# facebookresearch/goliath

Measured on AMD Instinct MI355X. Metric: relit views/sec (fwd+bwd) at 2048x1334, 250k Gaussians, higher is better.
Workload: dtype f32; 1 GPU; rgca_config2_envrelight; gaussians=250000, views_per_gpu=8, micro_batches=2, world_size=1, dist_backend=none, rccl_world_size=0, parallelism=view-parallel x1, launch=hip_graph_replay

## Files before the change

goliath_amd/csrc/gol_raster.h:

```cpp
#pragma once
#include <type_traits>

#include "gol_common.h"

namespace {

constexpr int kBatch = 256;
constexpr float kUnA = GOL_UN_A, kUnB = GOL_UN_B;
__device__ __forceinline__ float3 true_conic(float a, float b, float c) { return make_float3(a * kUnA, b * kUnB, c * kUnA); }
#ifdef GOL_EXACT_MATH
__device__ __forceinline__ float exact_sigma(float a, float b, float c, float dx, float dy) {
#pragma clang fp contract(off)
  const float t1 = (a * dx) * dx, t2 = (c * dy) * dy, t3 = (b * dx) * dy;
  const float h = 0.5f * (t1 + t2);
  return h + t3;
}
__device__ __forceinline__ float exact_exp_neg(float s) { return (float)exp(-(double)s); }
__device__ __forceinline__ float exact_next_T(float T, float alpha) {
#pragma clang fp contract(off)
  const float om = 1.f - alpha;
  return T * om;
}
#endif

struct TileCoord { int tile, tx, ty; bool ok; };

__device__ __forceinline__ TileCoord tile_of_block(int bid, int T, int tiles_x) {
  const int tiles_y = T / tiles_x;
  const int xcd = bid & 7, j = bid >> 3;
  TileCoord tc;
  const int row_local = j / tiles_x;
  tc.tx = j - row_local * tiles_x;
  tc.ty = row_local * 8 + xcd;
  tc.ok = tc.ty < tiles_y;
  tc.tile = tc.ty * tiles_x + tc.tx;
  return tc;
}

typedef float f1 __attribute__((ext_vector_type(1)));
typedef float f2 __attribute__((ext_vector_type(2)));
typedef int i1 __attribute__((ext_vector_type(1)));
typedef int i2 __attribute__((ext_vector_type(2)));

template <int PPL> struct Pix;
template <> struct Pix<2> { typedef f2 fv; typedef i2 iv; static constexpr int kWaves = 2; };
template <> struct Pix<1> { typedef f1 fv; typedef i1 iv; static constexpr int kWaves = 4; };

template <int PPL>
__device__ __forceinline__ void wave_rect(int wave, float tile_x0, float tile_y0, float& x0, float& x1, float& y0, float& y1) {
  if (PPL == 2) {
    x0 = tile_x0 + 0.5f; x1 = x0 + 15.f; y0 = tile_y0 + (float)(wave * 8) + 0.5f; y1 = y0 + 7.f;
  } else {
    x0 = tile_x0 + (float)((wave & 1) * 8) + 0.5f; x1 = x0 + 7.f; y0 = tile_y0 + (float)((wave >> 1) * 8) + 0.5f; y1 = y0 + 7.f;
  }
}

template <int PPL>
__device__ __forceinline__ int wave_mask(float gx, float gy, float ca, float cb, float cc, float tau, float ia, float ic,
                                         float exact, float tile_x0, float tile_y0) {
  constexpr int NW = Pix<PPL>::kWaves;
  if (!(tau >= 0.f)) return 0;
  if (exact == 0.f) return (1 << NW) - 1;
  int m = 0;
#pragma unroll
  for (int q = 0; q < NW; ++q) {
    float x0, x1, y0, y1;
    wave_rect<PPL>(q, tile_x0, tile_y0, x0, x1, y0, y1);
    const float ms = gol_min_sigma_rect(gx, gy, ca, cb, cc, ia, ic, x0, x1, y0, y1);
    m |= (ms <= tau) ? (1 << q) : 0;
  }
  return m;
}

template <int PPL>
__device__ __forceinline__ void lane_pixel(int tx, int ty, int wave, int lane, int& j, int& i0) {
  if (PPL == 2) { j = tx * 16 + (lane & 15); i0 = ty * 16 + wave * 8 + (lane >> 4) * 2; }
  else { j = tx * 16 + (wave & 1) * 8 + (lane & 7); i0 = ty * 16 + (wave >> 1) * 8 + (lane >> 3); }
}

struct __attribute__((aligned(16))) StagedRow { float4 a, b; float2 c; float2 pad; };

struct Staged { float4 a, b; float2 c; int mask; };
template <int PPL>
__device__ __forceinline__ Staged stage_entry(const float* __restrict__ records, size_t g, float tile_x0, float tile_y0) {
  const float4* R = reinterpret_cast<const float4*>(records + g * GOL_SPLAT_RECORD);
  const float4 q0 = R[0], q1 = R[1], q2 = R[2], q3 = R[3];
  Staged s;
  s.a = q0;
  s.b = q1;
  s.c = make_float2(q2.x, q2.y);
  const float3 cn = true_conic(q0.z, q0.w, q1.x);
  s.mask = wave_mask<PPL>(q0.x, q0.y, cn.x, cn.y, cn.z, q2.z, q2.w, q3.x, q3.y, tile_x0, tile_y0);
  return s;
}

template <typename V, int P>
__device__ __forceinline__ bool any_live(const V& live) {
  unsigned u = 0u;
#pragma unroll
  for (int q = 0; q < P; ++q) u |= __float_as_uint(live[q]);
  return u != 0u;
}

template <int PPL> using fvec = typename Pix<PPL>::fv;
template <int PPL> using ivec = typename Pix<PPL>::iv;

template <int PPL>
__device__ __forceinline__ void visit_falloff(float ca, float cb, float cc, float dx, const fvec<PPL>& dy, fvec<PPL>& sigma,
                                              fvec<PPL>& e) {
#ifndef GOL_EXACT_MATH
  sigma = (ca * dx * dx + cc * dy * dy) + (cb * dx) * dy;
#pragma unroll
  for (int q = 0; q < PPL; ++q) e[q] = __builtin_amdgcn_exp2f(-sigma[q]);
#else
#pragma unroll
  for (int q = 0; q < PPL; ++q) { sigma[q] = exact_sigma(ca, cb, cc, dx, dy[q]); e[q] = exact_exp_neg(sigma[q]); }
#endif
}

template <int PPL>
__device__ __forceinline__ unsigned long long fwd_step(const fvec<PPL>& sigma, fvec<PPL> alpha, const fvec<PPL>& live,
                                                       const fvec<PPL>& T_cur, fvec<PPL>& vis, fvec<PPL>& next_T,
                                                       bool (&take)[PPL], unsigned long long (&stop)[PPL]) {
  alpha *= live;
  vis = alpha * T_cur;
#ifndef GOL_EXACT_MATH
  next_T = T_cur - vis;
#else
#pragma unroll
  for (int q = 0; q < PPL; ++q) next_T[q] = exact_next_T(T_cur[q], alpha[q]);
#endif
  unsigned long long any_stop = 0ull;
#pragma unroll
  for (int q = 0; q < PPL; ++q) {
    const unsigned long long mc = gol_ballot(!(sigma[q] < 0.f)) & gol_ballot(!(alpha[q] < GOL_ALPHA_FLOOR));
    const unsigned long long ms = gol_ballot(next_T[q] <= GOL_T_STOP);
    take[q] = __builtin_amdgcn_inverse_ballot_w64(mc & ~ms);
    stop[q] = mc & ms;
    any_stop |= stop[q];
  }
  return any_stop;
}

template <int PPL>
__device__ __forceinline__ void fwd_take(const bool (&take)[PPL], const fvec<PPL>& next_T, fvec<PPL>& vis, fvec<PPL>& T_cur) {
#pragma unroll
  for (int q = 0; q < PPL; ++q) vis[q] = take[q] ? vis[q] : 0.f;
#ifndef GOL_EXACT_MATH
  T_cur -= vis;
#else
#pragma unroll
  for (int q = 0; q < PPL; ++q) T_cur[q] = take[q] ? next_T[q] : T_cur[q];
#endif
}

template <int PPL>
__device__ __forceinline__ unsigned long long bwd_taken(float opacity, const fvec<PPL>& e, const fvec<PPL>& sigma, int li,
                                                        const ivec<PPL>& bin_final, fvec<PPL>& alpha,
                                                        unsigned long long (&mv)[PPL]) {
  alpha = opacity * e;
  unsigned long long many = 0ull;
#pragma unroll
  for (int q = 0; q < PPL; ++q) {
    alpha[q] = fminf(GOL_ALPHA_CAP_BWD, alpha[q]);
    mv[q] = gol_ballot(li <= bin_final[q]) & gol_ballot(!(sigma[q] < 0.f)) & gol_ballot(!(alpha[q] < GOL_ALPHA_FLOOR));
    many |= mv[q];
  }
  return many;
}

template <int PPL>
__device__ __forceinline__ void bwd_recur(const unsigned long long (&mv)[PPL], fvec<PPL>& alpha, fvec<PPL>& T_cur,
                                          bool (&v)[PPL], fvec<PPL>& ra, fvec<PPL>& fac) {
#pragma unroll
  for (int q = 0; q < PPL; ++q) {
    v[q] = __builtin_amdgcn_inverse_ballot_w64(mv[q]);
    alpha[q] = v[q] ? alpha[q] : 0.f;
  }
  const fvec<PPL> one_m = 1.f - alpha;
#pragma unroll
  for (int q = 0; q < PPL; ++q) ra[q] = __builtin_amdgcn_rcpf(one_m[q]);
  const fvec<PPL> T_new = T_cur * ra;
  fac = alpha * T_new;
  T_cur = T_new;
}

template <int PPL>
__device__ __forceinline__ void bwd_moments(const fvec<PPL>& e, const fvec<PPL>& w, const fvec<PPL>& T_cur,
                                            const fvec<PPL>& ra, const fvec<PPL>& fac, const fvec<PPL>& tail,
                                            const bool (&v)[PPL], const fvec<PPL>& dy, fvec<PPL>& qsum, fvec<PPL>& gop,
                                            fvec<PPL>& gy, fvec<PPL>& gyy) {
  const fvec<PPL> v_alpha = T_cur * w + ra * (tail - qsum);
  qsum += fac * w;
  gop = e * v_alpha;
#pragma unroll
  for (int q = 0; q < PPL; ++q) gop[q] = v[q] ? gop[q] : 0.f;
  gy = gop * dy;
  gyy = gy * dy;
}
template <int PPL>
__device__ __forceinline__ float lane_sum(const fvec<PPL>& x) {
  float s = x[0];
#pragma unroll
  for (int q = 1; q < PPL; ++q) s += x[q];
  return s;
}

template <int PPL>
__device__ __forceinline__ int wave_last_entry(const ivec<PPL>& bin_final) {
  int wmax = bin_final[0];
#pragma unroll
  for (int q = 1; q < PPL; ++q) wmax = max(wmax, bin_final[q]);
#pragma unroll
  for (int off = 32; off > 0; off >>= 1) wmax = max(wmax, __shfl_xor(wmax, off, 64));
  return __builtin_amdgcn_readfirstlane(wmax);
}

inline int64_t raster_grid(int B, int img_h, int img_w) {
  return (int64_t)B * 8 * (((img_h + 15) / 16 + 7) / 8) * ((img_w + 15) / 16);
}

#define GOL_RASTER_CHECK_DIMS(bytes_per_pixel, too_large_msg)                                                           \
  do {                                                                                                                  \
    GOL_REQUIRE(B >= 0 && N >= 0, "negative size");                                                                     \
    GOL_REQUIRE(block == 16, "only block_width == 16 is implemented (the reference's value, render_gsplat.py:28)");     \
    GOL_REQUIRE(img_h > 0 && img_w > 0, "empty image");                                                                 \
    GOL_REQUIRE(raster_grid(B, img_h, img_w) < (1ll << 31), "too many tiles");                                          \
    GOL_REQUIRE((uint64_t)img_h * (uint64_t)img_w * (uint64_t)(bytes_per_pixel) < (1ull << 32), too_large_msg);         \
  } while (0)

template <typename F>
inline void with_ppl(int ppl, F&& fn) {
  if (ppl == 2) fn(std::integral_constant<int, 2>());
  else fn(std::integral_constant<int, 1>());
}
constexpr std::true_type kYes{}; constexpr std::false_type kNo{};

}
```

goliath_amd/csrc/raster.hip:

```cpp
#include <cstdlib>

#include "gol_raster.h"

namespace {

template <bool EXTRA, bool LAZY, int PPL>
__global__ __launch_bounds__(64 * Pix<PPL>::kWaves) void raster_fwd_kernel(
    int N, int img_h, int img_w, int planar, int tiles_x, int tiles_y, const int2* __restrict__ tile_bins,
    const int32_t* __restrict__ sorted_ids, int64_t capacity, const float* __restrict__ records,
    const float* __restrict__ background, float* __restrict__ out_img,
    float* __restrict__ out_extra, float* __restrict__ final_Ts, int32_t* __restrict__ final_idx,
    float* __restrict__ out_alpha, float* __restrict__ out_extra_norm, float norm_lo,
    const float* __restrict__ l1_target, const float* __restrict__ l1_mask, int l1_mask_c,
    uint8_t* __restrict__ l1_sign, float* __restrict__ l1_partial, int n_views) {
  typedef typename Pix<PPL>::fv fv;
  typedef typename Pix<PPL>::iv iv;
  constexpr int NW = Pix<PPL>::kWaves, NT = 64 * NW;
  __shared__ float s_l1[NW];
  __shared__ float4 s_a[kBatch];
  __shared__ float4 s_b[kBatch];
  __shared__ float2 s_c[kBatch];
  __shared__ int32_t s_mask[kBatch];
  const int T = tiles_x * tiles_y;
  const int view = blockIdx.x % n_views, slot = blockIdx.x / n_views;
  const TileCoord tc = tile_of_block(slot, T, tiles_x);
  if (!tc.ok) return;
  const int tid = threadIdx.x, lane = tid & 63, wave = tid >> 6;
  int j, i0;
  lane_pixel<PPL>(tc.tx, tc.ty, wave, lane, j, i0);
  bool in[PPL];
  fv py, live;
#pragma unroll
  for (int q = 0; q < PPL; ++q) {
    in[q] = (i0 + q < img_h) && (j < img_w);
    py[q] = (float)(i0 + q) + 0.5f;
    live[q] = in[q] ? 1.f : 0.f;
  }
  const float px = (float)j + 0.5f;

  const int2 range = tile_bins[(size_t)view * T + tc.tile];
  const int32_t* ids = sorted_ids + (size_t)view * capacity;
  const size_t goff = (size_t)view * N;

  fv T_cur = 1.f;
  iv cur_idx = 0;
  fv acc0 = 0.f, acc1 = 0.f, acc2 = 0.f, acc3 = 0.f;

  const int n_batches = (range.y - range.x + kBatch - 1) / kBatch;
  for (int bb = 0; bb < n_batches; ++bb) {
    if (__syncthreads_and(!any_live<fv, PPL>(live))) break;
    const int batch_start = range.x + bb * kBatch;
    for (int k = tid; k < kBatch; k += NT) {
      const int idx = batch_start + k;
      if (idx < range.y) {
        const Staged st = stage_entry<PPL>(records, goff + (size_t)ids[idx], (float)(tc.tx * 16), (float)(tc.ty * 16));
        s_a[k] = st.a; s_b[k] = st.b; s_c[k] = st.c; s_mask[k] = st.mask;
      } else {
        s_mask[k] = 0;
      }
    }
    __syncthreads();
    const int batch_size = min(kBatch, range.y - batch_start);
    for (int chunk = 0; chunk < batch_size; chunk += 64) {
      unsigned long long bits = gol_ballot((s_mask[chunk + lane] >> wave) & 1);
      if (LAZY && gol_ballot(any_live<fv, PPL>(live)) == 0ull) break;
      while (bits) {
        if (!LAZY && gol_ballot(any_live<fv, PPL>(live)) == 0ull) { chunk = batch_size; break; }
        const int t = chunk + __builtin_ctzll(bits);
        bits &= bits - 1;
        const float4 a4 = s_a[t];
        const float4 b4 = s_b[t];
        const float2 c2 = s_c[t];
        const float dx = a4.x - px;
        const fv dy = a4.y - py;
        fv sigma, e, alpha, vis, next_T;
        visit_falloff<PPL>(a4.z, a4.w, b4.x, dx, dy, sigma, e);
#pragma unroll
        for (int q = 0; q < PPL; ++q) alpha[q] = fminf(GOL_ALPHA_CAP_FWD, b4.y * e[q]);
        bool take[PPL];
        unsigned long long stop_m[PPL];
        const unsigned long long any_stop = fwd_step<PPL>(sigma, alpha, live, T_cur, vis, next_T, take, stop_m);
        bool half_done = false;
        if (!LAZY || any_stop != 0ull) {
#pragma unroll
          for (int q = 0; q < PPL; ++q) {
            const bool stop = __builtin_amdgcn_inverse_ballot_w64(stop_m[q]);
            live[q] = stop ? 0.f : live[q];
            if (LAZY) cur_idx[q] = stop ? (batch_start + t - 1) : cur_idx[q];
          }
          if (LAZY) half_done = gol_ballot(any_live<fv, PPL>(live)) == 0ull;
        }
        fwd_take<PPL>(take, next_T, vis, T_cur);
        acc0 += b4.z * vis; acc1 += b4.w * vis; acc2 += c2.x * vis;
        if (EXTRA) acc3 += c2.y * vis;
        if (!LAZY) {
#pragma unroll
          for (int q = 0; q < PPL; ++q) cur_idx[q] = take[q] ? (batch_start + t) : cur_idx[q];
        }
        if (LAZY && half_done) { chunk = batch_size; break; }
      }
    }
  }
  if (LAZY) {
#pragma unroll
    for (int q = 0; q < PPL; ++q) cur_idx[q] = live[q] != 0.f ? range.y - 1 : cur_idx[q];
  }

  const unsigned hw = (unsigned)img_h * (unsigned)img_w;
  const size_t vplane = (size_t)view * hw;
  float* __restrict__ o_T = final_Ts + vplane;
  int32_t* __restrict__ o_idx = final_idx + vplane;
  float* __restrict__ o_img = out_img + 3 * vplane;
  float* __restrict__ o_ex = (EXTRA && out_extra) ? out_extra + vplane : nullptr;
  float* __restrict__ o_alpha = out_alpha ? out_alpha + vplane : nullptr;
  float* __restrict__ o_norm = (EXTRA && out_extra_norm) ? out_extra_norm + vplane : nullptr;
  const float* __restrict__ i_tgt = l1_target ? l1_target + 3 * vplane : nullptr;
  const float* __restrict__ i_mask = l1_mask ? l1_mask + (size_t)l1_mask_c * vplane : nullptr;
  uint8_t* __restrict__ o_sign = l1_target ? l1_sign + vplane : nullptr;
  const float bg0 = background[0], bg1 = background[1], bg2 = background[2];
  float* __restrict__ o_img1 = o_img + (planar ? hw : 1u);
  float* __restrict__ o_img2 = o_img + (planar ? 2u * hw : 2u);
  const bool bwd_state = range.y > range.x;
  float l1_acc = 0.f;
#pragma unroll
  for (int q = 0; q < PPL; ++q) {
    if (!in[q]) continue;
    const unsigned pix = (unsigned)(i0 + q) * (unsigned)img_w + (unsigned)j;
    const unsigned b4 = pix * 4u;
    const unsigned bimg = planar ? b4 : 3u * b4;
    const float Tq = T_cur[q];
    const float c0 = acc0[q] + Tq * bg0, c1 = acc1[q] + Tq * bg1, c2 = acc2[q] + Tq * bg2, ex = acc3[q];
    *gol_at(o_T, b4) = Tq;
    if (bwd_state || !LAZY) *gol_at(o_idx, b4) = cur_idx[q];
    *gol_at(o_img, bimg) = c0; *gol_at(o_img1, bimg) = c1; *gol_at(o_img2, bimg) = c2;
    if (o_ex) *gol_at(o_ex, b4) = ex;
    if (o_alpha) *gol_at(o_alpha, b4) = 1.f - Tq;
    if (o_norm) *gol_at(o_norm, b4) = ex / fminf(fmaxf(1.f - Tq, norm_lo), 1.f);
    if (i_tgt) {
      const float m0 = i_mask ? *gol_at(i_mask, b4) : 1.f;
      const float cs[3] = {c0, c1, c2};
      unsigned code = 0u;
#pragma unroll
      for (int c = 0; c < 3; ++c) {
        const float m = (i_mask && l1_mask_c == 3) ? *gol_at(i_mask + (size_t)c * hw, b4) : m0;
        const float d = (cs[c] - *gol_at(i_tgt + (size_t)c * hw, b4)) * m;
        l1_acc += fabsf(d);
        code |= (d > 0.f ? 2u : (d < 0.f ? 0u : 1u)) << (2 * c);
      }
      if (bwd_state) *gol_at(o_sign, pix) = (uint8_t)code;
    }
  }
  if (l1_target) {
    const float ws = gol_wave_sum_to_lane63(l1_acc);
    if (lane == 63) s_l1[wave] = ws;
    __syncthreads();
    if (tid == 0) {
      float tot = 0.f;
#pragma unroll
      for (int w = 0; w < NW; ++w) tot += s_l1[w];
      l1_partial[(size_t)view * T + tc.tile] = tot;
    }
  }
}

__global__ __launch_bounds__(1024) void l1_sum_kernel(int n, const float* __restrict__ l1_partial, float scale,
                                                      float* __restrict__ l1_out) {
  __shared__ float s_w[16];
  float a0 = 0.f, a1 = 0.f, a2 = 0.f, a3 = 0.f;
  const int n4 = n >> 2;
  const float4* p4 = reinterpret_cast<const float4*>(l1_partial);
  int i = threadIdx.x;
  for (; i + 3 * 1024 < n4; i += 4 * 1024) {
    const float4 v0 = p4[i], v1 = p4[i + 1024], v2 = p4[i + 2048], v3 = p4[i + 3072];
    a0 += (v0.x + v0.y) + (v0.z + v0.w); a1 += (v1.x + v1.y) + (v1.z + v1.w);
    a2 += (v2.x + v2.y) + (v2.z + v2.w); a3 += (v3.x + v3.y) + (v3.z + v3.w);
  }
  for (; i < n4; i += 1024) { const float4 v = p4[i]; a0 += (v.x + v.y) + (v.z + v.w); }
  if ((int)threadIdx.x < (n & 3)) a1 += l1_partial[4 * n4 + threadIdx.x];
  const float ws = gol_wave_sum_to_lane63((a0 + a1) + (a2 + a3));
  if ((threadIdx.x & 63) == 63) s_w[threadIdx.x >> 6] = ws;
  __syncthreads();
  if (threadIdx.x == 0) {
    float tot = 0.f;
#pragma unroll
    for (int w = 0; w < 16; ++w) tot += s_w[w];
    l1_out[0] = tot * scale;
  }
}

constexpr int kBatchB = 64;
constexpr int kAcc = 12;

static_assert(kBatchB == 64, "raster_bwd_kernel ballots one 64-entry chunk per batch");

template <bool EXTRA, bool PACKED, int PPL>
__global__ __launch_bounds__(64 * Pix<PPL>::kWaves) void raster_bwd_kernel(
    int N, int img_h, int img_w, int planar, int tiles_x, int tiles_y, const int2* __restrict__ tile_bins,
    const int32_t* __restrict__ sorted_ids, int64_t capacity, const float* __restrict__ records,
    const float* __restrict__ background,
    const float* __restrict__ final_Ts, const int32_t* __restrict__ final_idx,
    const float* __restrict__ v_out_img, const float* __restrict__ v_out_extra,
    const float* __restrict__ v_out_alpha, float* __restrict__ v_xy, float* __restrict__ v_conic,
    float* __restrict__ v_colors, float* __restrict__ v_extra, float* __restrict__ v_opacity,
    const uint8_t* __restrict__ v_sign, const float* __restrict__ v_sign_mask, int v_sign_mask_c,
    const float* __restrict__ v_img_scale, float v_img_scale_mul, int n_views) {
  typedef typename Pix<PPL>::fv fv;
  typedef typename Pix<PPL>::iv iv;
  constexpr int NW = Pix<PPL>::kWaves, NT = 64 * NW;
  __shared__ StagedRow s_e[kBatchB];
  __shared__ int32_t s_mask[kBatchB];
  __shared__ int32_t s_id[kBatchB];
  __shared__ __attribute__((aligned(16))) float s_acc[NW][kBatchB][kAcc];
  __shared__ int32_t s_touched[NW][kBatchB];
  __shared__ int32_t s_wmax[NW];
  const int T = tiles_x * tiles_y;
  const int view = blockIdx.x % n_views, slot = blockIdx.x / n_views;
  const TileCoord tc = tile_of_block(slot, T, tiles_x);
  if (!tc.ok) return;
  const int2 range = tile_bins[(size_t)view * T + tc.tile];
  if (range.y <= range.x) return;
  const int tid = threadIdx.x, lane = tid & 63, wave = tid >> 6;
  int j, i0;
  lane_pixel<PPL>(tc.tx, tc.ty, wave, lane, j, i0);
  const float px = (float)j + 0.5f;
  const size_t hw = (size_t)img_h * img_w;
  const int32_t* ids = sorted_ids + (size_t)view * capacity;
  const size_t goff = (size_t)view * N;
  bool in[PPL];
  size_t pp[PPL];
  fv py, T_final;
  iv bin_final;
#pragma unroll
  for (int q = 0; q < PPL; ++q) {
    in[q] = (i0 + q < img_h) && (j < img_w);
    py[q] = (float)(i0 + q) + 0.5f;
    pp[q] = in[q] ? ((size_t)view * img_h + i0 + q) * img_w + j : 0;
    T_final[q] = in[q] ? final_Ts[pp[q]] : 1.f;
    bin_final[q] = in[q] ? final_idx[pp[q]] : (range.x - 1);
  }
  fv T_cur = T_final;
  fv vo0 = 0.f, vo1 = 0.f, vo2 = 0.f, vo3 = 0.f, voa = 0.f;
  {
    const float vsc = (v_img_scale ? v_img_scale[0] : 1.f) * v_img_scale_mul;
    const size_t os = planar ? hw : 1;
#pragma unroll
    for (int q = 0; q < PPL; ++q) {
      if (!in[q]) continue;
      const size_t p = pp[q];
      const int i = i0 + q;
      const size_t o = planar ? (size_t)view * 3 * hw + (size_t)i * img_w + j : 3 * p;
      float g0 = 0.f, g1 = 0.f, g2 = 0.f;
      if (v_out_img) { g0 = v_out_img[o]; g1 = v_out_img[o + os]; g2 = v_out_img[o + 2 * os]; }
      if (v_sign) {
        const unsigned code = v_sign[p];
        float m0 = vsc, m1 = vsc, m2 = vsc;
        if (v_sign_mask) {
          const float* mk = v_sign_mask + (size_t)view * v_sign_mask_c * hw + (size_t)i * img_w + j;
          m0 *= mk[0]; m1 *= (v_sign_mask_c == 3) ? mk[hw] : mk[0]; m2 *= (v_sign_mask_c == 3) ? mk[2 * hw] : mk[0];
        }
        g0 += (float)((int)(code & 3u) - 1) * m0;
        g1 += (float)((int)((code >> 2) & 3u) - 1) * m1;
        g2 += (float)((int)((code >> 4) & 3u) - 1) * m2;
      }
      vo0[q] = g0; vo1[q] = g1; vo2[q] = g2;
      if (EXTRA && v_out_extra) vo3[q] = v_out_extra[p];
      if (v_out_alpha) voa[q] = v_out_alpha[p];
    }
  }
  const fv tail = T_final * (voa - (background[0] * vo0 + background[1] * vo1 + background[2] * vo2));
  fv qsum = 0.f;

  const int wmax = wave_last_entry<PPL>(bin_final);
  if (lane == 0) s_wmax[wave] = wmax;
  __syncthreads();
  int bmax = s_wmax[0];
#pragma unroll
  for (int w = 1; w < NW; ++w) bmax = max(bmax, s_wmax[w]);
  bmax = min(bmax, range.y - 1);
  if (bmax < range.x) return;

  float* acc_lane = &s_acc[wave][0][lane >> 4];
  const int n_batches = (bmax - range.x + kBatchB) / kBatchB;
  auto entry_id = [&](int bb2) {
    const int e = bmax - bb2 * kBatchB - tid;
    return (tid < kBatchB && e >= range.x) ? ids[e] : 0;
  };
  int gid_next = entry_id(0);
  for (int bb = 0; bb < n_batches; ++bb) {
    __syncthreads();
    const int batch_end = bmax - bb * kBatchB;
    const int batch_size = min(kBatchB, batch_end + 1 - range.x);
    const int gid = gid_next;
    if (tid < kBatchB) {
      if (tid < batch_size) {
        const Staged st = stage_entry<PPL>(records, goff + (size_t)gid, (float)(tc.tx * 16), (float)(tc.ty * 16));
        s_e[tid].a = st.a; s_e[tid].b = st.b; s_e[tid].c = st.c; s_mask[tid] = st.mask;
        s_id[tid] = gid;
      } else {
        s_mask[tid] = 0;
      }
    }
    if (bb + 1 < n_batches) gid_next = entry_id(bb + 1);
    (&s_touched[0][0])[tid] = 0;
    __syncthreads();

    const int t0 = max(0, batch_end - wmax);
    unsigned long long bits = gol_ballot((s_mask[lane] >> wave) & 1);
    if (t0 > 0) bits &= ~0ull << t0;
    while (bits) {
      const int t = __builtin_ctzll(bits);
      bits &= bits - 1;
      const float4 a4 = s_e[t].a;
      const float4 b4 = s_e[t].b;
      const float2 c2 = s_e[t].c;
      const int li = batch_end - t;
      const float dx = a4.x - px;
      const fv dy = a4.y - py;
      fv sigma, vis, alpha, ra, fac;
      visit_falloff<PPL>(a4.z, a4.w, b4.x, dx, dy, sigma, vis);
      unsigned long long mv[PPL];
      if (bwd_taken<PPL>(b4.y, vis, sigma, li, bin_final, alpha, mv) == 0ull) continue;
      bool v[PPL];
      bwd_recur<PPL>(mv, alpha, T_cur, v, ra, fac);
      fv w = b4.z * vo0 + b4.w * vo1 + c2.x * vo2;
      if (EXTRA) w += c2.y * vo3;
      fv gop, gy, gyy;
      bwd_moments<PPL>(vis, w, T_cur, ra, fac, tail, v, dy, qsum, gop, gy, gyy);
      float g0s, g1s, g2s, g3 = 0.f;
      if (PPL == 2) {
        g0s = __builtin_fmaf(fac[0], vo0[0], fac[PPL - 1] * vo0[PPL - 1]);
        g1s = __builtin_fmaf(fac[0], vo1[0], fac[PPL - 1] * vo1[PPL - 1]);
        g2s = __builtin_fmaf(fac[0], vo2[0], fac[PPL - 1] * vo2[PPL - 1]);
        if (EXTRA) g3 = __builtin_fmaf(fac[0], vo3[0], fac[PPL - 1] * vo3[PPL - 1]);
      } else {
        g0s = fac[0] * vo0[0]; g1s = fac[0] * vo1[0]; g2s = fac[0] * vo2[0];
        if (EXTRA) g3 = fac[0] * vo3[0];
      }
      const float m0 = lane_sum<PPL>(gop), my = lane_sum<PPL>(gy), myy = lane_sum<PPL>(gyy);
      const float mx = m0 * dx, mxx = mx * dx, mxy = my * dx;
      const float r0 = gol_wave_sum4(g0s, g1s, g2s, m0);
      const float r1 = gol_wave_sum4(mx, my, mxx, mxy);
      const float r2 = gol_wave_sum_to_lane63(myy);
      const float r3 = EXTRA ? gol_wave_sum_to_lane63(g3) : 0.f;
      if ((lane & 15) == 15) {
        float* a = gol_at(acc_lane, (unsigned)t * (unsigned)(kAcc * sizeof(float)));
        a[0] = r0; a[4] = r1;
        if (lane == 63) { a[8 - 3] = r2; a[9 - 3] = r3; }
        s_touched[wave][t] = 1;
      }
    }
    __syncthreads();
    if (PACKED) {
      float* rec = v_colors;
      for (int idx = tid; idx < batch_size * 16; idx += NT) {
        const int t = idx >> 4, c = idx & 15;
        bool any = false;
#pragma unroll
        for (int w = 0; w < NW; ++w) any = any || (s_touched[w][t] != 0);
        if (!any || c > (EXTRA ? 9 : 8)) continue;
        const float4 a4 = s_e[t].a;
        const float4 b4 = s_e[t].b;
        const float nop = -b4.y, cc = b4.x;
        const int k1 = (c == 5) ? 4 : c, k2 = 5;
        const float w1 = (c == 4) ? nop * a4.z * kUnA : (c == 5) ? nop * a4.w * kUnB : (c == 6 || c == 8) ? 0.5f * nop
                       : (c == 7) ? nop : 1.f;
        const float w2 = (c == 4) ? nop * a4.w * kUnB : (c == 5) ? nop * cc * kUnA : 0.f;
        float s1 = 0.f, s2 = 0.f;
#pragma unroll
        for (int w = 0; w < NW; ++w) {
          const bool tw = s_touched[w][t] != 0;
          s1 += tw ? s_acc[w][t][k1] : 0.f;
          s2 += tw ? s_acc[w][t][k2] : 0.f;
        }
        atomicAdd(rec + (goff + (size_t)s_id[t]) * 16 + c, w1 * s1 + w2 * s2);
      }
    } else if (tid < batch_size) {
      float a[kAcc];
#pragma unroll
      for (int k = 0; k < kAcc; ++k) a[k] = 0.f;
      bool any = false;
#pragma unroll
      for (int w = 0; w < NW; ++w) {
        if (s_touched[w][tid]) {
          any = true;
          const float4* q = reinterpret_cast<const float4*>(&s_acc[w][tid][0]);
          const float4 q0 = q[0], q1 = q[1], q2 = q[2];
          a[0] += q0.x; a[1] += q0.y; a[2] += q0.z; a[3] += q0.w;
          a[4] += q1.x; a[5] += q1.y; a[6] += q1.z; a[7] += q1.w;
          a[8] += q2.x; a[9] += q2.y;
        }
      }
      if (any) {
        const size_t g = goff + (size_t)s_id[tid];
        const float4 a4 = s_e[tid].a;
        const float4 b4 = s_e[tid].b;
        const float nop = -b4.y;
        const float3 cn = true_conic(a4.z, a4.w, b4.x);
        atomicAdd(v_colors + 3 * g, a[0]); atomicAdd(v_colors + 3 * g + 1, a[1]); atomicAdd(v_colors + 3 * g + 2, a[2]);
        atomicAdd(v_opacity + g, a[3]);
        atomicAdd(v_xy + 2 * g, nop * (cn.x * a[4] + cn.y * a[5]));
        atomicAdd(v_xy + 2 * g + 1, nop * (cn.y * a[4] + cn.z * a[5]));
        atomicAdd(v_conic + 3 * g, 0.5f * nop * a[6]); atomicAdd(v_conic + 3 * g + 1, nop * a[7]);
        atomicAdd(v_conic + 3 * g + 2, 0.5f * nop * a[8]);
        if (EXTRA && v_extra) atomicAdd(v_extra + g, a[9]);
      }
    }
  }
}

__global__ __launch_bounds__(256) void raster_count_pairs_kernel(int N, int img_h, int img_w, int tiles_x, int tiles_y,
                                                                 const int2* __restrict__ tile_bins,
                                                                 const int32_t* __restrict__ sorted_ids, int64_t capacity,
                                                                 const float* __restrict__ records,
                                                                 const int32_t* __restrict__ final_idx,
                                                                 unsigned long long* __restrict__ counts) {
  __shared__ unsigned long long s_cnt[2];
  const int view = blockIdx.y, tile = blockIdx.x, T = tiles_x * tiles_y;
  const int ty = tile / tiles_x, tx = tile - ty * tiles_x;
  const int j = tx * 16 + (threadIdx.x & 15), i = ty * 16 + (threadIdx.x >> 4);
  if (threadIdx.x < 2) s_cnt[threadIdx.x] = 0ull;
  __syncthreads();
  const int2 range = tile_bins[(size_t)view * T + tile];
  unsigned long long tested = 0, taken = 0;
  if (i < img_h && j < img_w && range.y > range.x) {
    const int last = min(range.y - 1, final_idx[((size_t)view * img_h + i) * img_w + j]);
    const float px = (float)j + 0.5f, py = (float)i + 0.5f;
    for (int li = range.x; li <= last; ++li) {
      const float4* R = reinterpret_cast<const float4*>(records + ((size_t)view * N + sorted_ids[(size_t)view * capacity + li]) * GOL_SPLAT_RECORD);
      const float4 q0 = R[0], q1 = R[1];
      const float dx = q0.x - px, dy = q0.y - py;
      f1 sg, e;
      visit_falloff<1>(q0.z, q0.w, q1.x, dx, f1(dy), sg, e);
      const float alpha = fminf(GOL_ALPHA_CAP_FWD, q1.y * e[0]);
      ++tested;
      taken += (!(sg[0] < 0.f) && !(alpha < GOL_ALPHA_FLOOR)) ? 1 : 0;
    }
  }
  atomicAdd(&s_cnt[0], tested);
  atomicAdd(&s_cnt[1], taken);
  __syncthreads();
  if (threadIdx.x < 2 && s_cnt[threadIdx.x]) atomicAdd(counts + 2 * view + threadIdx.x, s_cnt[threadIdx.x]);
}

__global__ __launch_bounds__(256) void splat_pack_kernel(size_t n, const float* __restrict__ xys,
                                                         const float* __restrict__ conics,
                                                         const float* __restrict__ colors,
                                                         const float* __restrict__ extra,
                                                         const float* __restrict__ opacities,
                                                         float* __restrict__ records) {
  const size_t e = (size_t)blockIdx.x * 256 + threadIdx.x;
  if (e >= n) return;
  gol_record_write(records + e * GOL_SPLAT_RECORD, xys[2 * e], xys[2 * e + 1], conics[3 * e], conics[3 * e + 1],
                   conics[3 * e + 2], opacities[e], colors ? colors[3 * e] : 0.f, colors ? colors[3 * e + 1] : 0.f,
                   colors ? colors[3 * e + 2] : 0.f, extra ? extra[e] : 0.f);
}

}

extern "C" int gol_raster_plan(int B, int* fwd_pixels_per_lane) {
  static const int forced = getenv("GOL_RASTER_PPL") ? atoi(getenv("GOL_RASTER_PPL")) : 0;
  if (fwd_pixels_per_lane) *fwd_pixels_per_lane = (forced == 1 || forced == 2) ? forced : (B <= 2 ? 1 : 2);
  return GOL_OK;
}

extern "C" int gol_raster_count_pairs(int B, int N, int img_h, int img_w, const int32_t* tile_bins, const int32_t* sorted_ids,
                                      int64_t capacity, const float* records, const int32_t* final_idx, uint64_t* counts,
                                      void* stream) {
  GOL_REQUIRE(B >= 0 && N >= 0 && img_h > 0 && img_w > 0, "bad size");
  if (B == 0) return GOL_OK;
  GOL_REQUIRE(tile_bins && final_idx && counts && (capacity == 0 || sorted_ids) && (N == 0 || records), "null pointer");
  hipStream_t s = (hipStream_t)stream;
  if (hipMemsetAsync(counts, 0, sizeof(uint64_t) * 2 * (size_t)B, s) != hipSuccess) {
    gol_set_error("gol_raster_count_pairs: hipMemsetAsync failed");
    return GOL_ERR_LAUNCH;
  }
  const int tiles_x = (img_w + 15) / 16, tiles_y = (img_h + 15) / 16;
  raster_count_pairs_kernel<<<dim3(tiles_x * tiles_y, B), 256, 0, s>>>(
      N, img_h, img_w, tiles_x, tiles_y, reinterpret_cast<const int2*>(tile_bins), sorted_ids, capacity, records, final_idx,
      reinterpret_cast<unsigned long long*>(counts));
  GOL_CHECK_LAUNCH();
  return GOL_OK;
}

extern "C" int gol_splat_pack(int B, int N, const float* xys, const float* conics, const float* colors,
                              const float* extra, const float* opacities, float* records, void* stream) {
  GOL_REQUIRE(B >= 0 && N >= 0, "negative size");
  if (B == 0 || N == 0) return GOL_OK;
  GOL_REQUIRE(xys && conics && opacities && records, "null pointer");
  const size_t n = (size_t)B * N;
  splat_pack_kernel<<<gol_cdiv((long long)n, 256), 256, 0, (hipStream_t)stream>>>(n, xys, conics, colors, extra, opacities,
                                                                                 records);
  GOL_CHECK_LAUNCH();
  return GOL_OK;
}

extern "C" int gol_rasterize_fwd(int B, int N, int img_h, int img_w, int block, int planar, const int32_t* tile_bins,
                                 const int32_t* sorted_ids, int64_t capacity, const float* records, int with_extra,
                                 const float* background, float* out_img,
                                 float* out_extra, float* final_Ts, int32_t* final_idx, float* out_alpha,
                                 float* out_extra_norm, float norm_lo, const float* l1_target, const float* l1_mask,
                                 int l1_mask_c, uint8_t* l1_sign, float* l1_partial, float* l1_out, float l1_scale,
                                 int pixels_per_lane, void* stream) {
  GOL_RASTER_CHECK_DIMS(12, "image too large (32-bit byte offsets inside a view)");
  if (B == 0) return GOL_OK;
  GOL_REQUIRE(tile_bins && background && out_img && final_Ts && final_idx, "null pointer");
  GOL_REQUIRE(capacity == 0 || sorted_ids, "null sorted_ids");
  GOL_REQUIRE(N == 0 || records, "null Gaussian records");
  GOL_REQUIRE((!out_extra && !out_extra_norm) || with_extra || N == 0, "out_extra / out_extra_norm need the extra channel");
  GOL_REQUIRE(!with_extra || out_extra || out_extra_norm, "extra without an output for it");
  GOL_REQUIRE(!l1_target || (planar && l1_sign && l1_partial), "the fused L1 needs planar images, l1_sign and l1_partial");
  GOL_REQUIRE(!l1_mask || (l1_target && (l1_mask_c == 1 || l1_mask_c == 3)), "l1_mask: 1 or 3 channels, with l1_target");
  GOL_REQUIRE(!l1_out || l1_target, "l1_out needs l1_target");
  const int tiles_x = (img_w + 15) / 16, tiles_y = (img_h + 15) / 16;
  const dim3 grid((unsigned)raster_grid(B, img_h, img_w));
  const int2* bins = reinterpret_cast<const int2*>(tile_bins);
  hipStream_t s = (hipStream_t)stream;
  GOL_REQUIRE(pixels_per_lane >= 0 && pixels_per_lane <= 2, "pixels_per_lane: 0 (choose by B), 1 or 2");
  int ppl = pixels_per_lane;
  if (ppl == 0) gol_raster_plan(B, &ppl);
  auto launch = [&](auto ex_c, auto lazy_c) {
    with_ppl(ppl, [&](auto ppl_c) {
      constexpr bool EX = decltype(ex_c)::value, LZ = decltype(lazy_c)::value;
      constexpr int PPL = decltype(ppl_c)::value;
      raster_fwd_kernel<EX, LZ, PPL><<<grid, 64 * Pix<PPL>::kWaves, 0, s>>>(
          N, img_h, img_w, planar, tiles_x, tiles_y, bins, sorted_ids, capacity, records, background, out_img, out_extra,
          final_Ts, final_idx, out_alpha, EX ? out_extra_norm : nullptr, norm_lo, l1_target, l1_mask, l1_mask_c, l1_sign,
          l1_partial, B);
    });
  };
  const bool ex = out_extra || out_extra_norm;
  if (ex && planar) launch(kYes, kYes);
  else if (ex) launch(kYes, kNo);
  else if (planar) launch(kNo, kYes);
  else launch(kNo, kNo);
  if (l1_out) l1_sum_kernel<<<1, 1024, 0, s>>>(B * tiles_x * tiles_y, l1_partial, l1_scale, l1_out);
  GOL_CHECK_LAUNCH();
  return GOL_OK;
}

extern "C" int gol_rasterize_bwd(int B, int N, int img_h, int img_w, int block, int planar, const int32_t* tile_bins,
                                 const int32_t* sorted_ids, int64_t capacity, const float* records, int with_extra,
                                 const float* background, const float* final_Ts,
                                 const int32_t* final_idx, const float* v_out_img, const float* v_out_extra,
                                 const float* v_out_alpha, float* v_xy, float* v_conic, float* v_colors,
                                 float* v_extra, float* v_opacity, int grad_stride, const uint8_t* v_sign,
                                 const float* v_sign_mask, int v_sign_mask_c, const float* v_img_scale,
                                 float v_img_scale_mul, int pixels_per_lane, void* stream) {
  GOL_RASTER_CHECK_DIMS(0, "");
  if (B == 0 || N == 0 || capacity == 0) return GOL_OK;
  GOL_REQUIRE(tile_bins && sorted_ids && background && final_Ts && final_idx, "null pointer");
  GOL_REQUIRE(v_out_img || v_sign, "no upstream image gradient (v_out_img or v_sign)");
  GOL_REQUIRE(!v_sign || planar, "the sign image of the fused L1 goes with planar images");
  GOL_REQUIRE(!v_sign_mask || (v_sign && (v_sign_mask_c == 1 || v_sign_mask_c == 3)), "v_sign_mask: 1 or 3 channels, with v_sign");
  GOL_REQUIRE(records, "null Gaussian records");
  GOL_REQUIRE(v_xy && v_conic && v_colors && v_opacity, "null gradient output");
  GOL_REQUIRE(!(v_out_extra || v_extra) || with_extra, "extra-channel gradients need the extra channel");
  GOL_REQUIRE(grad_stride == 0 || grad_stride == GOL_GRAD_RECORD, "grad_stride must be 0 (dense arrays) or 16 (records)");
  const bool packed = grad_stride == GOL_GRAD_RECORD;
  if (packed)
    GOL_REQUIRE(v_opacity == v_colors + 3 && v_xy == v_colors + 4 && v_conic == v_colors + 6 &&
                    (!v_extra || v_extra == v_colors + 9),
                "record layout is [rgb | opacity | xy | conic | extra | pad] (GOL_GRAD_RECORD floats)");
  const int tiles_x = (img_w + 15) / 16, tiles_y = (img_h + 15) / 16;
  const dim3 grid((unsigned)raster_grid(B, img_h, img_w));
  const int2* bins = reinterpret_cast<const int2*>(tile_bins);
  hipStream_t s = (hipStream_t)stream;
  GOL_REQUIRE(pixels_per_lane >= 0 && pixels_per_lane <= 2, "pixels_per_lane: 0 (2), 1 or 2");
  const int ppl = pixels_per_lane ? pixels_per_lane : 2;
  const bool ex = with_extra && (v_out_extra || v_extra);
  auto launch = [&](auto ex_c, auto packed_c) {
    with_ppl(ppl, [&](auto ppl_c) {
      constexpr bool EX = decltype(ex_c)::value, PK = decltype(packed_c)::value;
      constexpr int PPL = decltype(ppl_c)::value;
      raster_bwd_kernel<EX, PK, PPL><<<grid, 64 * Pix<PPL>::kWaves, 0, s>>>(
          N, img_h, img_w, planar, tiles_x, tiles_y, bins, sorted_ids, capacity, records, background, final_Ts, final_idx,
          v_out_img, EX ? v_out_extra : nullptr, v_out_alpha, v_xy, v_conic, v_colors, EX ? v_extra : nullptr, v_opacity,
          v_sign, v_sign_mask, v_sign_mask_c, v_img_scale, v_img_scale_mul, B);
    });
  };
  if (ex && packed) launch(kYes, kYes);
  else if (ex) launch(kYes, kNo);
  else if (packed) launch(kNo, kYes);
  else launch(kNo, kNo);
  GOL_CHECK_LAUNCH();
  return GOL_OK;
}
```

goliath_amd/csrc/raster_nd.hip:

```cpp
#include "gol_raster.h"

namespace {

constexpr int kChunkMax = 16;
constexpr int kBatchNdB = 64;

template <int CK>
__device__ __forceinline__ void stage_colors(float* __restrict__ row, const float* __restrict__ colors, size_t g, int C,
                                             int c0, int nc) {
  const float* col = colors + g * (size_t)C + c0;
#pragma unroll
  for (int c = 0; c < CK; ++c) row[c] = (c < nc) ? col[c] : 0.f;
}

template <int CK, int PPL>
__global__ __launch_bounds__(64 * Pix<PPL>::kWaves) void raster_nd_fwd_kernel(
    int N, int C, int c_first, int img_h, int img_w, int tiles_x, int tiles_y, const int2* __restrict__ tile_bins,
    const int32_t* __restrict__ sorted_ids, int64_t capacity, const float* __restrict__ records,
    const float* __restrict__ colors, const float* __restrict__ background, float* __restrict__ out_img,
    float* __restrict__ final_Ts, int32_t* __restrict__ final_idx, int n_views) {
  typedef typename Pix<PPL>::fv fv;
  typedef typename Pix<PPL>::iv iv;
  constexpr int NW = Pix<PPL>::kWaves, NT = 64 * NW;
  __shared__ float4 s_a[kBatch];
  __shared__ float2 s_b[kBatch];
  __shared__ int32_t s_mask[kBatch];
  __shared__ __attribute__((aligned(16))) float s_col[kBatch * CK];
  const int T = tiles_x * tiles_y;
  const int view = blockIdx.x % n_views, slot = blockIdx.x / n_views;
  const TileCoord tc = tile_of_block(slot, T, tiles_x);
  if (!tc.ok) return;
  const int c0 = c_first + (int)blockIdx.y * CK;
  const int nc = min(CK, C - c0);
  const int tid = threadIdx.x, lane = tid & 63, wave = tid >> 6;
  int j, i0;
  lane_pixel<PPL>(tc.tx, tc.ty, wave, lane, j, i0);
  bool in[PPL];
  fv py, live;
#pragma unroll
  for (int q = 0; q < PPL; ++q) {
    in[q] = (i0 + q < img_h) && (j < img_w);
    py[q] = (float)(i0 + q) + 0.5f;
    live[q] = in[q] ? 1.f : 0.f;
  }
  const float px = (float)j + 0.5f;

  const int2 range = tile_bins[(size_t)view * T + tc.tile];
  const int32_t* ids = sorted_ids + (size_t)view * capacity;
  const size_t goff = (size_t)view * N;

  fv T_cur = 1.f;
  iv cur_idx = 0;
  fv acc[CK];
#pragma unroll
  for (int c = 0; c < CK; ++c) acc[c] = 0.f;

  const int n_batches = (range.y - range.x + kBatch - 1) / kBatch;
  for (int bb = 0; bb < n_batches; ++bb) {
    if (__syncthreads_and(!any_live<fv, PPL>(live))) break;
    const int batch_start = range.x + bb * kBatch;
    for (int k = tid; k < kBatch; k += NT) {
      const int idx = batch_start + k;
      if (idx < range.y) {
        const size_t g = goff + (size_t)ids[idx];
        const Staged st = stage_entry<PPL>(records, g, (float)(tc.tx * 16), (float)(tc.ty * 16));
        s_a[k] = st.a; s_b[k] = make_float2(st.b.x, st.b.y); s_mask[k] = st.mask;
        stage_colors<CK>(s_col + k * CK, colors, g, C, c0, nc);
      } else {
        s_mask[k] = 0;
      }
    }
    __syncthreads();
    const int batch_size = min(kBatch, range.y - batch_start);
    for (int chunk = 0; chunk < batch_size; chunk += 64) {
      unsigned long long bits = gol_ballot((s_mask[chunk + lane] >> wave) & 1);
      while (bits) {
        if (gol_ballot(any_live<fv, PPL>(live)) == 0ull) { chunk = batch_size; break; }
        const int t = chunk + __builtin_ctzll(bits);
        bits &= bits - 1;
        const float4 a4 = s_a[t];
        const float2 b2 = s_b[t];
        const float dx = a4.x - px;
        const fv dy = a4.y - py;
        fv sigma, e, alpha, vis, next_T;
        visit_falloff<PPL>(a4.z, a4.w, b2.x, dx, dy, sigma, e);
#pragma unroll
        for (int q = 0; q < PPL; ++q) alpha[q] = fminf(GOL_ALPHA_CAP_FWD, b2.y * e[q]);
        bool take[PPL];
        unsigned long long stop_m[PPL];
        fwd_step<PPL>(sigma, alpha, live, T_cur, vis, next_T, take, stop_m);
#pragma unroll
        for (int q = 0; q < PPL; ++q) live[q] = __builtin_amdgcn_inverse_ballot_w64(stop_m[q]) ? 0.f : live[q];
        fwd_take<PPL>(take, next_T, vis, T_cur);
        const float* col = s_col + t * CK;
#pragma unroll
        for (int c = 0; c < CK; ++c) acc[c] += col[c] * vis;
#pragma unroll
        for (int q = 0; q < PPL; ++q) cur_idx[q] = take[q] ? (batch_start + t) : cur_idx[q];
      }
    }
  }

  const unsigned hw = (unsigned)img_h * (unsigned)img_w;
  const size_t vplane = (size_t)view * hw;
  float* __restrict__ o_img = out_img + (size_t)C * vplane + c0;
  float* __restrict__ o_T = final_Ts + vplane;
  int32_t* __restrict__ o_idx = final_idx + vplane;
  const bool first = c0 == 0;
  float bg[CK];
#pragma unroll
  for (int c = 0; c < CK; ++c) bg[c] = (c < nc) ? background[c0 + c] : 0.f;
#pragma unroll
  for (int q = 0; q < PPL; ++q) {
    if (!in[q]) continue;
    const unsigned pix = (unsigned)(i0 + q) * (unsigned)img_w + (unsigned)j;
    const float Tq = T_cur[q];
    if (first) { *gol_at(o_T, pix * 4u) = Tq; *gol_at(o_idx, pix * 4u) = cur_idx[q]; }
    const unsigned bimg = pix * (unsigned)C * 4u;
#pragma unroll
    for (int c = 0; c < CK; ++c)
      if (c < nc) *gol_at(o_img + c, bimg) = acc[c][q] + Tq * bg[c];
  }
}

template <int CK, int PPL>
__global__ __launch_bounds__(64 * Pix<PPL>::kWaves) void raster_nd_bwd_kernel(
    int N, int C, int c_first, int img_h, int img_w, int tiles_x, int tiles_y, const int2* __restrict__ tile_bins,
    const int32_t* __restrict__ sorted_ids, int64_t capacity, const float* __restrict__ records,
    const float* __restrict__ colors, const float* __restrict__ background, const float* __restrict__ final_Ts,
    const int32_t* __restrict__ final_idx, const float* __restrict__ v_out_img, const float* __restrict__ v_out_alpha,
    float* __restrict__ v_xy, float* __restrict__ v_conic, float* __restrict__ v_colors, float* __restrict__ v_opacity,
    int n_views) {
  typedef typename Pix<PPL>::fv fv;
  typedef typename Pix<PPL>::iv iv;
  constexpr int NW = Pix<PPL>::kWaves, NT = 64 * NW;
  constexpr int NS = CK + 6, NG = (NS + 3) / 4, kRow = 4 * NG;
  static_assert(NW * kBatchNdB == NT, "s_touched is cleared one element per thread");
  __shared__ float4 s_a[kBatchNdB];
  __shared__ float2 s_b[kBatchNdB];
  __shared__ int32_t s_mask[kBatchNdB];
  __shared__ int32_t s_id[kBatchNdB];
  __shared__ __attribute__((aligned(16))) float s_col[kBatchNdB * CK];
  __shared__ __attribute__((aligned(16))) float s_acc[NW][kBatchNdB][kRow];
  __shared__ int32_t s_touched[NW][kBatchNdB];
  __shared__ int32_t s_wmax[NW];
  const int T = tiles_x * tiles_y;
  const int view = blockIdx.x % n_views, slot = blockIdx.x / n_views;
  const TileCoord tc = tile_of_block(slot, T, tiles_x);
  if (!tc.ok) return;
  const int2 range = tile_bins[(size_t)view * T + tc.tile];
  if (range.y <= range.x) return;
  const int c0 = c_first + (int)blockIdx.y * CK;
  const int nc = min(CK, C - c0);
  const int tid = threadIdx.x, lane = tid & 63, wave = tid >> 6;
  int j, i0;
  lane_pixel<PPL>(tc.tx, tc.ty, wave, lane, j, i0);
  const float px = (float)j + 0.5f;
  const int32_t* ids = sorted_ids + (size_t)view * capacity;
  const size_t goff = (size_t)view * N;
  fv py, T_final, voa = 0.f;
  iv bin_final;
  fv vo[CK];
#pragma unroll
  for (int c = 0; c < CK; ++c) vo[c] = 0.f;
#pragma unroll
  for (int q = 0; q < PPL; ++q) {
    const bool in = (i0 + q < img_h) && (j < img_w);
    py[q] = (float)(i0 + q) + 0.5f;
    const size_t p = in ? ((size_t)view * img_h + i0 + q) * img_w + j : 0;
    T_final[q] = in ? final_Ts[p] : 1.f;
    bin_final[q] = in ? final_idx[p] : (range.x - 1);
    if (in) {
      const float* g = v_out_img + p * (size_t)C + c0;
#pragma unroll
      for (int c = 0; c < CK; ++c) vo[c][q] = (c < nc) ? g[c] : 0.f;
      if (v_out_alpha && c0 == 0) voa[q] = v_out_alpha[p];
    }
  }

  const int wmax = wave_last_entry<PPL>(bin_final);
  if (lane == 0) s_wmax[wave] = wmax;
  __syncthreads();
  int bmax = s_wmax[0];
#pragma unroll
  for (int w = 1; w < NW; ++w) bmax = max(bmax, s_wmax[w]);
  bmax = min(bmax, range.y - 1);
  if (bmax < range.x) return;

  fv bgdot = 0.f;
#pragma unroll
  for (int c = 0; c < CK; ++c) bgdot += ((c < nc) ? background[c0 + c] : 0.f) * vo[c];
  const fv tail = T_final * (voa - bgdot);
  fv T_cur = T_final;
  fv qsum = 0.f;

  float* acc_lane = &s_acc[wave][0][lane >> 4];
  const int n_batches = (bmax - range.x + kBatchNdB) / kBatchNdB;
  for (int bb = 0; bb < n_batches; ++bb) {
    __syncthreads();
    const int batch_end = bmax - bb * kBatchNdB;
    const int batch_size = min(kBatchNdB, batch_end + 1 - range.x);
    if (tid < kBatchNdB) {
      if (tid < batch_size) {
        const int gid = ids[batch_end - tid];
        const size_t g = goff + (size_t)gid;
        const Staged st = stage_entry<PPL>(records, g, (float)(tc.tx * 16), (float)(tc.ty * 16));
        s_a[tid] = st.a; s_b[tid] = make_float2(st.b.x, st.b.y); s_mask[tid] = st.mask;
        s_id[tid] = gid;
        stage_colors<CK>(s_col + tid * CK, colors, g, C, c0, nc);
      } else {
        s_mask[tid] = 0;
      }
    }
    (&s_touched[0][0])[tid] = 0;
    __syncthreads();

    const int t0 = max(0, batch_end - wmax);
    unsigned long long bits = gol_ballot((s_mask[lane] >> wave) & 1);
    if (t0 > 0) bits &= ~0ull << t0;
    while (bits) {
      const int t = __builtin_ctzll(bits);
      bits &= bits - 1;
      const float4 a4 = s_a[t];
      const float2 b2 = s_b[t];
      const int li = batch_end - t;
      const float dx = a4.x - px;
      const fv dy = a4.y - py;
      fv sigma, vis, alpha, ra, fac;
      visit_falloff<PPL>(a4.z, a4.w, b2.x, dx, dy, sigma, vis);
      unsigned long long mv[PPL];
      if (bwd_taken<PPL>(b2.y, vis, sigma, li, bin_final, alpha, mv) == 0ull) continue;
      bool v[PPL];
      bwd_recur<PPL>(mv, alpha, T_cur, v, ra, fac);
      const float* col = s_col + t * CK;
      fv w = 0.f;
#pragma unroll
      for (int c = 0; c < CK; ++c) w += col[c] * vo[c];
      fv gop, gy, gyy;
      bwd_moments<PPL>(vis, w, T_cur, ra, fac, tail, v, dy, qsum, gop, gy, gyy);
      float s[kRow];
#pragma unroll
      for (int c = 0; c < CK; ++c) {
        s[c] = fac[0] * vo[c][0];
#pragma unroll
        for (int q = 1; q < PPL; ++q) s[c] = __builtin_fmaf(fac[q], vo[c][q], s[c]);
      }
      const float m0 = lane_sum<PPL>(gop), my = lane_sum<PPL>(gy), myy = lane_sum<PPL>(gyy);
      const float mx = m0 * dx;
      s[CK + 0] = m0; s[CK + 1] = mx; s[CK + 2] = my; s[CK + 3] = mx * dx; s[CK + 4] = my * dx; s[CK + 5] = myy;
#pragma unroll
      for (int k = NS; k < kRow; ++k) s[k] = 0.f;
      float r[NG];
#pragma unroll
      for (int gi = 0; gi < NG; ++gi) r[gi] = gol_wave_sum4(s[4 * gi], s[4 * gi + 1], s[4 * gi + 2], s[4 * gi + 3]);
      if ((lane & 15) == 15) {
        float* a = gol_at(acc_lane, (unsigned)t * (unsigned)(kRow * sizeof(float)));
#pragma unroll
        for (int gi = 0; gi < NG; ++gi) a[4 * gi] = r[gi];
        s_touched[wave][t] = 1;
      }
    }
    __syncthreads();
    for (int idx = tid; idx < batch_size * NS; idx += NT) {
      const int t = idx / NS, k = idx - t * NS;
      if (k < CK && k >= nc) continue;
      bool any = false;
#pragma unroll
      for (int w = 0; w < NW; ++w) any = any || (s_touched[w][t] != 0);
      if (!any) continue;
      const size_t g = goff + (size_t)s_id[t];
      const float4 a4 = s_a[t];
      const float2 b2 = s_b[t];
      const float nop = -b2.y;
      const float3 cn = true_conic(a4.z, a4.w, b2.x);
      const float ca = cn.x, cb = cn.y, cc = cn.z;
      int k1 = k, k2 = k;
      float w1 = 1.f, w2 = 0.f;
      float* dst;
      if (k < CK) {
        dst = v_colors + g * (size_t)C + c0 + k;
      } else {
        const int m = k - CK;
        k1 = (m == 1 || m == 2) ? CK + 1 : k;
        k2 = CK + 2;
        w1 = (m == 0) ? 1.f : (m == 1) ? nop * ca : (m == 2) ? nop * cb : (m == 4) ? nop : 0.5f * nop;
        w2 = (m == 1) ? nop * cb : (m == 2) ? nop * cc : 0.f;
        dst = (m == 0) ? v_opacity + g : (m <= 2) ? v_xy + 2 * g + (m - 1) : v_conic + 3 * g + (m - 3);
      }
      float s1 = 0.f, s2 = 0.f;
#pragma unroll
      for (int w = 0; w < NW; ++w) {
        const bool tw = s_touched[w][t] != 0;
        s1 += tw ? s_acc[w][t][k1] : 0.f;
        s2 += tw ? s_acc[w][t][k2] : 0.f;
      }
      atomicAdd(dst, w1 * s1 + w2 * s2);
    }
  }
}

struct NdPlan { int n16, tail, tail_first; };
NdPlan nd_plan(int C) {
  const int r = C % kChunkMax;
  NdPlan p;
  p.n16 = C / kChunkMax + (r > 8 ? 1 : 0);
  p.tail = (r == 0 || r > 8) ? 0 : r <= 1 ? 1 : r <= 2 ? 2 : r <= 4 ? 4 : 8;
  p.tail_first = (C / kChunkMax) * kChunkMax;
  return p;
}

template <typename F>
bool for_nd_launches(int C, F&& fn) {
  const NdPlan pl = nd_plan(C);
  if (pl.n16 > 0) fn(std::integral_constant<int, 16>(), pl.n16, 0);
  switch (pl.tail) {
    case 0: break;
    case 1: fn(std::integral_constant<int, 1>(), 1, pl.tail_first); break;
    case 2: fn(std::integral_constant<int, 2>(), 1, pl.tail_first); break;
    case 4: fn(std::integral_constant<int, 4>(), 1, pl.tail_first); break;
    case 8: fn(std::integral_constant<int, 8>(), 1, pl.tail_first); break;
    default: return false;
  }
  return true;
}

}

extern "C" int gol_rasterize_nd_fwd(int B, int N, int C, int img_h, int img_w, int block, const int32_t* tile_bins,
                                    const int32_t* sorted_ids, int64_t capacity, const float* records, const float* colors,
                                    const float* background, float* out_img, float* final_Ts, int32_t* final_idx,
                                    int pixels_per_lane, void* stream) {
  GOL_REQUIRE(C >= 1, "C >= 1 colour channels");
  GOL_REQUIRE(C <= 16 * 65535, "too many colour channels (at most 1048560: one launch row of 16-channel chunks)");
  GOL_RASTER_CHECK_DIMS((uint64_t)C * 4ull, "image too large (32-bit byte offsets inside a view: H * W * C * 4 bytes)");
  if (B == 0) return GOL_OK;
  GOL_REQUIRE(tile_bins && background && out_img && final_Ts && final_idx, "null pointer");
  GOL_REQUIRE(capacity == 0 || sorted_ids, "null sorted_ids");
  GOL_REQUIRE(N == 0 || (records && colors), "null Gaussian records / colors");
  GOL_REQUIRE(pixels_per_lane >= 0 && pixels_per_lane <= 2, "pixels_per_lane: 0 (choose by B), 1 or 2");
  int ppl = pixels_per_lane;
  if (ppl == 0) gol_raster_plan(B, &ppl);
  const int tiles_x = (img_w + 15) / 16, tiles_y = (img_h + 15) / 16;
  const unsigned gx = (unsigned)raster_grid(B, img_h, img_w);
  const int2* bins = reinterpret_cast<const int2*>(tile_bins);
  hipStream_t s = (hipStream_t)stream;
  const bool covered = for_nd_launches(C, [&](auto ck_c, int n_chunks, int c_first) {
    with_ppl(ppl, [&](auto ppl_c) {
      constexpr int CK = decltype(ck_c)::value, PPL = decltype(ppl_c)::value;
      raster_nd_fwd_kernel<CK, PPL><<<dim3(gx, n_chunks), 64 * Pix<PPL>::kWaves, 0, s>>>(
          N, C, c_first, img_h, img_w, tiles_x, tiles_y, bins, sorted_ids, capacity, records, colors, background, out_img,
          final_Ts, final_idx, B);
    });
  });
  GOL_REQUIRE(covered, "no kernel instance for this chunk width");
  GOL_CHECK_LAUNCH();
  return GOL_OK;
}

extern "C" int gol_rasterize_nd_bwd(int B, int N, int C, int img_h, int img_w, int block, const int32_t* tile_bins,
                                    const int32_t* sorted_ids, int64_t capacity, const float* records, const float* colors,
                                    const float* background, const float* final_Ts, const int32_t* final_idx,
                                    const float* v_out_img, const float* v_out_alpha, float* v_xy, float* v_conic,
                                    float* v_colors, float* v_opacity, void* stream) {
  GOL_REQUIRE(C >= 1, "C >= 1 colour channels");
  GOL_REQUIRE(C <= 16 * 65535, "too many colour channels (at most 1048560: one launch row of 16-channel chunks)");
  GOL_RASTER_CHECK_DIMS((uint64_t)C * 4ull, "image too large (32-bit byte offsets inside a view: H * W * C * 4 bytes)");
  if (B == 0 || N == 0 || capacity == 0) return GOL_OK;
  GOL_REQUIRE(tile_bins && sorted_ids && background && final_Ts && final_idx, "null pointer");
  GOL_REQUIRE(v_out_img, "null v_out_img");
  GOL_REQUIRE(records && colors, "null Gaussian records / colors");
  GOL_REQUIRE(v_xy && v_conic && v_colors && v_opacity, "null gradient output");
  const int tiles_x = (img_w + 15) / 16, tiles_y = (img_h + 15) / 16;
  const unsigned gx = (unsigned)raster_grid(B, img_h, img_w);
  const int2* bins = reinterpret_cast<const int2*>(tile_bins);
  hipStream_t s = (hipStream_t)stream;
  const bool covered = for_nd_launches(C, [&](auto ck_c, int n_chunks, int c_first) {
    constexpr int CK = decltype(ck_c)::value;
    raster_nd_bwd_kernel<CK, 2><<<dim3(gx, n_chunks), 128, 0, s>>>(
        N, C, c_first, img_h, img_w, tiles_x, tiles_y, bins, sorted_ids, capacity, records, colors, background, final_Ts,
        final_idx, v_out_img, v_out_alpha, v_xy, v_conic, v_colors, v_opacity, B);
  });
  GOL_REQUIRE(covered, "no kernel instance for this chunk width");
  GOL_CHECK_LAUNCH();
  return GOL_OK;
}
```

goliath_amd/csrc/render.hip:

```cpp
#include <cstring>

#include "gol_common.h"

namespace {
inline int64_t align256(int64_t x) { return (x + 255) & ~(int64_t)255; }
template <typename T>
inline T* at(void* ws, int64_t off) { return reinterpret_cast<T*>(reinterpret_cast<char*>(ws) + off); }
}

static int render_layout(int B, int N, int img_h, int img_w, int64_t capacity, int with_l1, bool projected, gol_render_ws* L) {
  GOL_REQUIRE(B >= 0 && N >= 0 && img_h > 0 && img_w > 0 && capacity >= 0 && L != nullptr, "bad argument");
  const int64_t T = (int64_t)((img_w + 15) / 16) * ((img_h + 15) / 16), P = (int64_t)img_h * img_w;
  const int64_t BN = (int64_t)B * N, cap = capacity > 0 ? capacity : 1;
  int64_t o = 0;
  auto take = [&](int64_t bytes) { const int64_t at_ = o; o = align256(o + bytes); return at_; };
  L->cov3d = -1;
  L->xys = projected ? -1 : take(BN * 2 * 4);
  L->depths = projected ? -1 : take(BN * 4);
  L->radii = projected ? -1 : take(BN * 4);
  L->conics = projected ? -1 : take(BN * 3 * 4);
  L->comp = projected ? -1 : take(BN * 4);
  L->nth = -1;
  L->opac_eff = projected ? -1 : take(BN * 4);
  L->records = projected ? -1 : take(BN * GOL_SPLAT_RECORD * 4);
  L->tile_count = take((int64_t)B * T * 4);
  L->tile_bins = take((int64_t)B * T * 2 * 4);
  L->keys = take((int64_t)B * cap * 8);
  L->sorted_ids = take((int64_t)B * cap * 4);
  L->n_isect = take((int64_t)B * 4);
  L->final_T = take((int64_t)B * P * 4);
  L->final_idx = take((int64_t)B * P * 4);
  L->l1_sign = with_l1 ? take((int64_t)B * P) : -1;
  L->total = o;
  return GOL_OK;
}

extern "C" int gol_render_layout(int B, int N, int img_h, int img_w, int64_t capacity, int with_l1, gol_render_ws* L) {
  return render_layout(B, N, img_h, img_w, capacity, with_l1, false, L);
}

extern "C" int gol_render_layout_projected(int B, int N, int img_h, int img_w, int64_t capacity, int with_l1,
                                           gol_render_ws* L) {
  return render_layout(B, N, img_h, img_w, capacity, with_l1, true, L);
}

static int render_fwd_from(int B, int N, int img_h, int img_w, const float* xys, const float* depths, const int32_t* radii,
                           const float* conics, const float* opac_eff, const float* records, const float* background,
                           int with_depth, float norm_lo, int64_t capacity, void* ws, const gol_render_ws* L,
                           float* out_img, float* out_depth, float* out_alpha, float* out_depth_norm,
                           const float* l1_target, const float* l1_mask, int l1_mask_c, float* l1_partial, float* l1_out,
                           float l1_scale, void* stream) {
  int rc = gol_bin_sort(B, N, xys, depths, radii, conics, opac_eff, img_h, img_w, 16, capacity,
                        at<int32_t>(ws, L->tile_count), at<int32_t>(ws, L->tile_bins), at<uint64_t>(ws, L->keys),
                        at<int32_t>(ws, L->sorted_ids), at<int32_t>(ws, L->n_isect), nullptr, stream);
  if (rc != GOL_OK) return rc;
  return gol_rasterize_fwd(B, N, img_h, img_w, 16, 1, at<int32_t>(ws, L->tile_bins), at<int32_t>(ws, L->sorted_ids),
                           capacity, records, with_depth ? 1 : 0, background, out_img,
                           with_depth ? out_depth : nullptr, at<float>(ws, L->final_T), at<int32_t>(ws, L->final_idx),
                           out_alpha, with_depth ? out_depth_norm : nullptr, norm_lo, l1_target, l1_mask, l1_mask_c,
                           l1_target ? at<uint8_t>(ws, L->l1_sign) : nullptr, l1_partial, l1_out, l1_scale, 0,
                           stream);
}

static int render_bwd_to_records(int B, int N, int img_h, int img_w, const float* records, const float* background,
                                 int64_t capacity, void* ws, const gol_render_ws* L, const float* v_img,
                                 const float* v_depth, const float* v_alpha, int use_l1_sign, const float* l1_mask,
                                 int l1_mask_c, const float* v_img_scale, float v_img_scale_mul, float* grad_records,
                                 void* stream) {
  hipStream_t s = (hipStream_t)stream;
  if (hipMemsetAsync(grad_records, 0, sizeof(float) * (size_t)B * N * GOL_GRAD_RECORD, s) != hipSuccess) {
    gol_set_error("gol_render_bwd: hipMemsetAsync failed");
    return GOL_ERR_LAUNCH;
  }
  float* g = grad_records;
  const bool use_depth = v_depth != nullptr;
  return gol_rasterize_bwd(B, N, img_h, img_w, 16, 1, at<int32_t>(ws, L->tile_bins), at<int32_t>(ws, L->sorted_ids),
                           capacity, records, use_depth ? 1 : 0, background,
                           at<float>(ws, L->final_T), at<int32_t>(ws, L->final_idx), v_img, v_depth, v_alpha, g + 4, g + 6,
                           g, use_depth ? g + 9 : nullptr, g + 3, GOL_GRAD_RECORD,
                           use_l1_sign ? at<uint8_t>(ws, L->l1_sign) : nullptr, use_l1_sign ? l1_mask : nullptr,
                           use_l1_sign ? l1_mask_c : 0, v_img_scale, v_img_scale_mul, 0, stream);
}

extern "C" int gol_render_fwd(int B, int N, int img_h, int img_w, float glob_scale, float clip_thresh, const float* means,
                              const float* scales, const float* quats, const float* opacity, const float* colors,
                              const float* viewmats, const float* intrins, const float* background, int with_depth,
                              float norm_lo, int64_t capacity, void* workspace, const gol_render_ws* L, float* out_img,
                              float* out_depth, float* out_alpha, float* out_depth_norm, const float* l1_target,
                              const float* l1_mask, int l1_mask_c, float* l1_partial, float* l1_out, float l1_scale,
                              void* stream) {
  GOL_REQUIRE(workspace != nullptr && L != nullptr, "null workspace / layout");
  GOL_REQUIRE(!l1_target || L->l1_sign >= 0, "layout was computed without the fused L1");
  if (B == 0) return GOL_OK;
  void* ws = workspace;
  GOL_REQUIRE(!l1_out || l1_target, "l1_out needs l1_target");
  int rc = gol_project_fwd(B, N, means, scales, glob_scale, quats, viewmats, intrins, img_h, img_w, 16, clip_thresh,
                           nullptr, at<float>(ws, L->xys), at<float>(ws, L->depths),
                           at<int32_t>(ws, L->radii), at<float>(ws, L->conics), at<float>(ws, L->comp),
                           nullptr, opacity, at<float>(ws, L->opac_eff), colors,
                           at<float>(ws, L->records), stream);
  if (rc != GOL_OK) return rc;
  return render_fwd_from(B, N, img_h, img_w, at<float>(ws, L->xys), at<float>(ws, L->depths), at<int32_t>(ws, L->radii),
                         at<float>(ws, L->conics), at<float>(ws, L->opac_eff), at<float>(ws, L->records), background,
                         with_depth, norm_lo, capacity, ws, L, out_img, out_depth, out_alpha, out_depth_norm, l1_target,
                         l1_mask, l1_mask_c, l1_partial, l1_out, l1_scale, stream);
}

extern "C" int gol_render_fwd_projected(int B, int N, const gol_shade_proj* proj, const float* background, int with_depth,
                                        float norm_lo, int64_t capacity, void* workspace, const gol_render_ws* L,
                                        float* out_img, float* out_depth, float* out_alpha, float* out_depth_norm,
                                        const float* l1_target, const float* l1_mask, int l1_mask_c, float* l1_partial,
                                        float* l1_out, float l1_scale, void* stream) {
  GOL_REQUIRE(workspace != nullptr && L != nullptr && proj != nullptr, "null workspace / layout / projection");
  GOL_REQUIRE(!l1_target || L->l1_sign >= 0, "layout was computed without the fused L1");
  GOL_REQUIRE(!l1_out || l1_target, "l1_out needs l1_target");
  if (B == 0) return GOL_OK;
  return render_fwd_from(B, N, proj->img_h, proj->img_w, proj->xys, proj->depths, proj->radii, proj->conics,
                         proj->opac_eff, proj->records, background, with_depth, norm_lo, capacity, workspace, L, out_img,
                         out_depth, out_alpha, out_depth_norm, l1_target, l1_mask, l1_mask_c, l1_partial, l1_out,
                         l1_scale, stream);
}

extern "C" int gol_render_bwd(int B, int N, int img_h, int img_w, float glob_scale, const float* means,
                              const float* scales, const float* quats, const float* opacity, const float* viewmats,
                              const float* intrins, const float* background, int64_t capacity, void* workspace,
                              const gol_render_ws* L, const float* v_img, const float* v_depth, const float* v_alpha,
                              int use_l1_sign, const float* l1_mask, int l1_mask_c, const float* v_img_scale,
                              float v_img_scale_mul, float* grad_records, float* v_mean, float* v_scale, float* v_quat, float* v_opacity,
                              float* v_colors, void* stream) {
  GOL_REQUIRE(workspace != nullptr && L != nullptr && grad_records != nullptr, "null workspace / layout / gradient records");
  GOL_REQUIRE(!use_l1_sign || L->l1_sign >= 0, "layout was computed without the fused L1");
  if (B == 0 || N == 0) return GOL_OK;
  void* ws = workspace;
  const float* g = grad_records;
  const bool use_depth = v_depth != nullptr;
  int rc = render_bwd_to_records(B, N, img_h, img_w, at<float>(ws, L->records), background, capacity, ws, L, v_img, v_depth,
                                 v_alpha, use_l1_sign, l1_mask, l1_mask_c, v_img_scale, v_img_scale_mul, grad_records,
                                 stream);
  if (rc != GOL_OK) return rc;
  return gol_project_bwd_records(B, N, means, scales, glob_scale, quats, viewmats, intrins, at<int32_t>(ws, L->radii),
                                 at<float>(ws, L->conics), at<float>(ws, L->comp), opacity, g, use_depth ? 1 : 0, v_mean,
                                 v_scale, v_quat, v_opacity, v_colors, stream);
}

extern "C" int gol_render_bwd_projected(int B, int N, const gol_shade_proj* proj, const float* background, int64_t capacity,
                                        void* workspace, const gol_render_ws* L, const float* v_img, const float* v_depth,
                                        const float* v_alpha, int use_l1_sign, const float* l1_mask, int l1_mask_c,
                                        const float* v_img_scale, float v_img_scale_mul, float* grad_records,
                                        void* stream) {
  GOL_REQUIRE(workspace != nullptr && L != nullptr && proj != nullptr && grad_records != nullptr,
              "null workspace / layout / projection / gradient records");
  GOL_REQUIRE(!use_l1_sign || L->l1_sign >= 0, "layout was computed without the fused L1");
  if (B == 0 || N == 0) return GOL_OK;
  return render_bwd_to_records(B, N, proj->img_h, proj->img_w, proj->records, background, capacity, workspace, L, v_img,
                               v_depth, v_alpha, use_l1_sign, l1_mask, l1_mask_c, v_img_scale, v_img_scale_mul,
                               grad_records, stream);
}
```

goliath_amd/splat.py:

```python
import ctypes
import math
import os

import torch

from . import _lib, views as _views
from ._lib import c_float, c_i64, c_int, fptr, ptr, stream_ptr

BLOCK = 16
GRAD_RECORD = 16
SPLAT_RECORD = 16

def _tiles(img_h, img_w, block=BLOCK):
    return ((img_w + block - 1) // block) * ((img_h + block - 1) // block)


class CapacityPlanner:

    def __init__(self):
        self.capacity = {}
        self.mode = os.environ.get("GOLIATH_CAPACITY_MODE", "adaptive")
        self.pending = []
        self.frozen = False
        self.frozen_log = []
        self.reruns = 0
        self.truncated = 0
        self.last_worst = {}
        self.force_block = set()
        self._pinned = {}

    def check_frozen(self):
        for n_isect, capacity in self.frozen_log:
            worst = int(n_isect.max()) if n_isect.numel() else 0
            if worst > capacity:
                raise _lib.GoliathHipError(f"a captured render_views call overflowed its intersection capacity "
                                           f"({worst} > {capacity}): re-capture with a larger capacity")

    def must_block(self, key):
        if self.mode == "verify" or os.environ.get("GOLIATH_STRICT_CAPACITY", "0") == "1":
            return True
        if self.mode == "async":
            return False
        seen, cap = self.last_worst.get(key), self.capacity.get(key)
        return key in self.force_block or seen is None or cap is None or seen * 1.5 > cap

    def passed(self, key):
        self.force_block.discard(key)

    def get(self, key):
        return self.capacity.get(key)

    def initial(self, N, T):
        return int(min(2**31 - 1, max(1 << 16, 16 * N + T)))

    def set(self, key, counts_max):
        want = int(min(2**31 - 1, max(1 << 16, int(counts_max * 2.0) + 4096)))
        self.capacity[key] = max(self.capacity.get(key, 0), want)
        return self.capacity[key]

    def observe(self, key, worst, capacity):
        self.last_worst[key] = worst
        if key not in self.capacity or worst * 1.5 > capacity:
            self.set(key, worst)

    def _take_pinned(self, B):
        free = self._pinned.setdefault(B, [])
        return free.pop() if free else torch.empty(B, dtype=torch.int32, pin_memory=True)

    def fetch(self, n_isect):
        B = n_isect.numel()
        host = self._take_pinned(B)
        host.copy_(n_isect, non_blocking=True)
        ev = torch.cuda.Event()
        ev.record()
        return host, ev

    def finish(self, host, ev):
        ev.synchronize()
        worst = int(host.max()) if host.numel() else 0
        self._pinned[host.numel()].append(host)
        return worst

    def note(self, key, n_isect, capacity):
        host, ev = self.fetch(n_isect)
        self.pending.append((ev, host, capacity, key))

    def poll(self, block=False):
        still, overflow = [], None
        for ev, host, capacity, key in self.pending:
            if block:
                ev.synchronize()
            if ev.query():
                worst = int(host.max()) if host.numel() else 0
                self._pinned[host.numel()].append(host)
                if worst > capacity:
                    self.last_worst[key] = worst
                    self.set(key, worst)
                    self.force_block.add(key)
                    overflow = (worst, capacity, key)
                else:
                    self.observe(key, worst, capacity)
            else:
                still.append((ev, host, capacity, key))
        self.pending = still
        if overflow is not None:
            worst, capacity, key = overflow
            msg = (f"a previous render_views call overflowed its intersection capacity ({worst} > {capacity}): its tile "
                   f"lists were truncated. Capacity was raised to {self.capacity[key]}")
            if self.mode == "async":
                raise _lib.GoliathHipError(msg + " -- re-run the step (GOLIATH_CAPACITY_MODE=verify repairs inside the "
                                                 "call instead).")
            import sys
            import warnings

            self.truncated += 1
            try:
                frame = sys._getframe(2)
            except ValueError:
                frame = sys._getframe(0)
            warnings.warn_explicit(msg + "; calls of this shape check their own counts before returning until one has passed "
                                         "(GOLIATH_CAPACITY_MODE=verify checks every call).", CapacityWarning,
                                   frame.f_code.co_filename, frame.f_lineno, module=frame.f_globals.get("__name__"), registry={})


class CapacityWarning(RuntimeWarning):
    """A render_views call was found, after the fact, to have rendered with truncated tile lists (adaptive mode)."""


PLANNER = CapacityPlanner()


class _Workspace:

    def __init__(self, B, N, T, capacity, device):
        self.capacity = capacity
        self.tile_count = torch.zeros(B, T, dtype=torch.int32, device=device)
        self.tile_bins = torch.empty(B, T, 2, dtype=torch.int32, device=device)
        self.keys = torch.empty(B, max(capacity, 1), dtype=torch.int64, device=device)
        self.sorted_ids = torch.empty(B, max(capacity, 1), dtype=torch.int32, device=device)
        self.n_isect = torch.empty(B, dtype=torch.int32, device=device)
        self.reach = torch.empty(B, max(N, 1), dtype=torch.int64, device=device)


_F32, _I32, _I64, _U8 = torch.float32, torch.int32, torch.int64, torch.uint8


def _p(x, dtype=_F32, name="tensor"):
    return ctypes.c_void_p(x) if x is None or isinstance(x, int) else ptr(x, dtype, name)


def _abi_bin_sort(*, B, N, xys, depths, radii, conics=None, opacities=None, img_h, img_w, capacity, tile_count, tile_bins,
                  isect_keys, sorted_ids, n_isect, reach_scratch=None):
    _lib.call("gol_bin_sort", c_int(B), c_int(N), _p(xys), _p(depths), _p(radii, _I32), _p(conics), _p(opacities),
              c_int(img_h), c_int(img_w), c_int(BLOCK), c_i64(capacity), _p(tile_count, _I32), _p(tile_bins, _I32),
              _p(isect_keys, _I64), _p(sorted_ids, _I32), _p(n_isect, _I32), _p(reach_scratch, _I64), stream_ptr())


def _abi_project_fwd(*, B, N, means3d, scales, glob_scale, quats, viewmats, intrins, img_h, img_w, clip_thresh, cov3d=None,
                     xys, depths, radii, conics, compensation, num_tiles_hit=None, opacities=None, opac_eff=None,
                     colors=None, records=None):
    _lib.call("gol_project_fwd", c_int(B), c_int(N), _p(means3d, name="means3d"), _p(scales, name="scales"),
              c_float(glob_scale), _p(quats, name="quats"), _p(viewmats, name="viewmat"), _p(intrins, name="intrins"),
              c_int(img_h), c_int(img_w), c_int(BLOCK), c_float(clip_thresh), _p(cov3d), _p(xys), _p(depths),
              _p(radii, _I32), _p(conics), _p(compensation), _p(num_tiles_hit, _I32), _p(opacities, name="opacity"),
              _p(opac_eff), _p(colors, name="colors"), _p(records), stream_ptr())


def _abi_project_bwd(*, B, N, means3d, scales, glob_scale, quats, viewmats, intrins, cov3d=None, radii, conics, compensation,
                     v_xy=None, v_depth=None, v_conic=None, v_compensation=None, opacities=None, v_opac_eff=None,
                     grad_stride=0, v_mean3d, v_scale, v_quat, v_opacity=None):
    _lib.call("gol_project_bwd", c_int(B), c_int(N), _p(means3d), _p(scales), c_float(glob_scale), _p(quats),
              _p(viewmats), _p(intrins), _p(cov3d), _p(radii, _I32), _p(conics), _p(compensation), _p(v_xy), _p(v_depth),
              _p(v_conic), _p(v_compensation), _p(opacities), _p(v_opac_eff), c_int(grad_stride), _p(v_mean3d),
              _p(v_scale), _p(v_quat), _p(v_opacity), stream_ptr())


def _abi_rasterize_fwd(*, B, N, img_h, img_w, planar, tile_bins, sorted_ids, capacity, records, with_extra, background,
                       out_img, out_extra=None, final_Ts, final_idx, out_alpha=None, out_extra_norm=None, norm_lo=0.0,
                       l1_target=None, l1_mask=None, l1_mask_c=0, l1_sign=None, l1_partial=None, l1_out=None,
                       l1_scale=1.0, pixels_per_lane=0):
    _lib.call("gol_rasterize_fwd", c_int(B), c_int(N), c_int(img_h), c_int(img_w), c_int(BLOCK), c_int(planar),
              _p(tile_bins, _I32), _p(sorted_ids, _I32), c_i64(capacity), _p(records), c_int(with_extra),
              _p(background), _p(out_img), _p(out_extra), _p(final_Ts), _p(final_idx, _I32), _p(out_alpha),
              _p(out_extra_norm), c_float(norm_lo), _p(l1_target), _p(l1_mask), c_int(l1_mask_c), _p(l1_sign, _U8),
              _p(l1_partial), _p(l1_out), c_float(l1_scale), c_int(pixels_per_lane), stream_ptr())


def _abi_rasterize_bwd(*, B, N, img_h, img_w, planar, tile_bins, sorted_ids, capacity, records, with_extra, background,
                       final_Ts, final_idx, v_out_img=None, v_out_extra=None, v_out_alpha=None, v_xy, v_conic, v_colors,
                       v_extra=None, v_opacity, grad_stride=0, v_sign=None, v_sign_mask=None, v_sign_mask_c=0,
                       v_img_scale=None, v_img_scale_mul=1.0, pixels_per_lane=0):
    _lib.call("gol_rasterize_bwd", c_int(B), c_int(N), c_int(img_h), c_int(img_w), c_int(BLOCK), c_int(planar),
              _p(tile_bins, _I32), _p(sorted_ids, _I32), c_i64(capacity), _p(records), c_int(with_extra), _p(background),
              _p(final_Ts), _p(final_idx, _I32), _p(v_out_img), _p(v_out_extra), _p(v_out_alpha), _p(v_xy), _p(v_conic),
              _p(v_colors), _p(v_extra), _p(v_opacity), c_int(grad_stride), _p(v_sign, _U8), _p(v_sign_mask),
              c_int(v_sign_mask_c), _p(v_img_scale), c_float(v_img_scale_mul), c_int(pixels_per_lane), stream_ptr())


def _abi_rasterize_nd_fwd(*, B, N, C, img_h, img_w, tile_bins, sorted_ids, capacity, records, colors, background, out_img,
                          final_Ts, final_idx, pixels_per_lane=0):
    _lib.call("gol_rasterize_nd_fwd", c_int(B), c_int(N), c_int(C), c_int(img_h), c_int(img_w), c_int(BLOCK),
              _p(tile_bins, _I32), _p(sorted_ids, _I32), c_i64(capacity), _p(records), _p(colors), _p(background),
              _p(out_img), _p(final_Ts), _p(final_idx, _I32), c_int(pixels_per_lane), stream_ptr())


def _abi_rasterize_nd_bwd(*, B, N, C, img_h, img_w, tile_bins, sorted_ids, capacity, records, colors, background, final_Ts,
                          final_idx, v_out_img, v_out_alpha=None, v_xy, v_conic, v_colors, v_opacity):
    _lib.call("gol_rasterize_nd_bwd", c_int(B), c_int(N), c_int(C), c_int(img_h), c_int(img_w), c_int(BLOCK),
              _p(tile_bins, _I32), _p(sorted_ids, _I32), c_i64(capacity), _p(records), _p(colors), _p(background),
              _p(final_Ts), _p(final_idx, _I32), _p(v_out_img), _p(v_out_alpha), _p(v_xy), _p(v_conic), _p(v_colors),
              _p(v_opacity), stream_ptr())


def _bin_sort(B, N, xys, depths, radii, img_h, img_w, ws, conics=None, opacities=None):
    _abi_bin_sort(B=B, N=N, xys=xys, depths=depths, radii=radii, conics=conics, opacities=opacities, img_h=img_h,
                  img_w=img_w, capacity=ws.capacity, tile_count=ws.tile_count, tile_bins=ws.tile_bins, isect_keys=ws.keys,
                  sorted_ids=ws.sorted_ids, n_isect=ws.n_isect, reach_scratch=ws.reach)


def _project_fwd(B, N, means, scales, glob_scale, quats, viewmats, intrins, img_h, img_w, clip,
                 opacities=None, colors=None):
    f = dict(dtype=torch.float32, device=means.device)
    records = torch.empty(B, N, SPLAT_RECORD, **f) if colors is not None else None
    cov3d, xys, conics = (torch.empty(B, N, k, **f) for k in (6, 2, 3))
    depths, comp = torch.empty(B, N, **f), torch.empty(B, N, **f)
    radii, nth = (torch.empty(B, N, dtype=torch.int32, device=means.device) for _ in range(2))
    opac_eff = torch.empty(B, N, **f) if opacities is not None else None
    _abi_project_fwd(B=B, N=N, means3d=means, scales=scales, glob_scale=glob_scale, quats=quats, viewmats=viewmats,
                     intrins=intrins, img_h=img_h, img_w=img_w, clip_thresh=clip, cov3d=cov3d, xys=xys, depths=depths,
                     radii=radii, conics=conics, compensation=comp, num_tiles_hit=nth, opacities=opacities,
                     opac_eff=opac_eff, colors=colors, records=records)
    out = (cov3d, xys, depths, radii, conics, comp, nth, opac_eff)
    return out + (records,) if colors is not None else out


def _pack_records(B, N, xys, conics, colors, extra, opacities):
    records = torch.empty(B, N, SPLAT_RECORD, dtype=torch.float32, device=xys.device)
    _lib.call("gol_splat_pack", c_int(B), c_int(N), fptr(xys), fptr(conics), fptr(colors), fptr(extra), fptr(opacities),
              fptr(records), stream_ptr())
    return records


def _f32c(t):
    return t.to(torch.float32).contiguous()


class _ProjectGaussians(torch.autograd.Function):
    @staticmethod
    def forward(ctx, means3d, scales, glob_scale, quats, viewmat, fx, fy, cx, cy, img_height, img_width,
                block_width, clip_thresh):
        if block_width != BLOCK:
            raise NotImplementedError("goliath_amd implements block_width=16 (the reference's value)")
        N = means3d.shape[0]
        dev = means3d.device
        means3d, scales, quats = _f32c(means3d), _f32c(scales), _f32c(quats)
        vm = _f32c(viewmat).reshape(-1)[:12].contiguous().view(1, 12)
        intr = torch.tensor([[fx, fy, cx, cy]], dtype=torch.float32).to(dev, non_blocking=True)
        with _lib.device_guard(dev):
            cov3d, xys, depths, radii, conics, comp, nth, _ = _project_fwd(
                1, N, means3d, scales, float(glob_scale), quats, vm, intr, img_height, img_width,
                float(clip_thresh))
        ctx.save_for_backward(means3d, scales, quats, vm, intr, cov3d[0], radii[0], conics[0], comp[0])
        ctx.glob_scale = float(glob_scale)
        ctx.set_materialize_grads(False)
        outs = (xys[0], depths[0], radii[0], conics[0], comp[0], nth[0], cov3d[0])
        ctx.mark_non_differentiable(outs[2], outs[5])
        return outs

    @staticmethod
    def backward(ctx, v_xys, v_depths, v_radii, v_conics, v_compensation, v_num_tiles_hit, v_cov3d):
        means3d, scales, quats, vm, intr, cov3d, radii, conics, comp = ctx.saved_tensors
        N = means3d.shape[0]
        v_mean = torch.empty_like(means3d)
        v_scale = torch.empty_like(scales)
        v_quat = torch.empty_like(quats)
        c = lambda t: None if t is None else _f32c(t)
        g_xy, g_depth, g_conic, g_comp = c(v_xys), c(v_depths), c(v_conics), c(v_compensation)
        with _lib.device_guard(means3d.device):
            _abi_project_bwd(B=1, N=N, means3d=means3d, scales=scales, glob_scale=ctx.glob_scale, quats=quats, viewmats=vm,
                             intrins=intr, cov3d=cov3d, radii=radii, conics=conics, compensation=comp, v_xy=g_xy,
                             v_depth=g_depth, v_conic=g_conic, v_compensation=g_comp, v_mean3d=v_mean, v_scale=v_scale,
                             v_quat=v_quat)
        return (v_mean, v_scale, None, v_quat) + (None,) * 9



def project_gaussians(means3d, scales, glob_scale, quats, viewmat, fx, fy, cx, cy, img_height, img_width,
                      block_width, clip_thresh=0.01):
    if means3d.dim() != 2 or means3d.shape[1] != 3:
        raise ValueError("means3d must have dimensions (N, 3)")
    return _ProjectGaussians.apply(means3d, scales, glob_scale, quats, viewmat, fx, fy, cx, cy, img_height,
                                   img_width, block_width, clip_thresh)


class _RasterizeGaussians(torch.autograd.Function):
    @staticmethod
    def forward(ctx, xys, depths, radii, conics, num_tiles_hit, colors, opacity, img_height, img_width,
                block_width, background, return_alpha):
        dev = xys.device
        N, C = xys.shape[0], colors.shape[-1]
        xys, depths, conics, colors = _f32c(xys), _f32c(depths), _f32c(conics), _f32c(colors)
        opacity = _f32c(opacity).reshape(-1)
        radii = radii.to(torch.int32).contiguous()
        background = _f32c(background)
        n_isect = int(num_tiles_hit.to(torch.int64).sum().item()) if N > 0 else 0
        ctx.n_isect = n_isect
        ctx.dims = (img_height, img_width)
        if n_isect < 1:
            out_img = torch.ones(img_height, img_width, C, device=dev) * background
            final_Ts = torch.zeros(img_height, img_width, device=dev)
            ctx.save_for_backward(xys, conics, colors, opacity, background)
        else:
            T = _tiles(img_height, img_width)
            ws = _Workspace(1, N, T, n_isect, dev)
            out_img = torch.empty(1, img_height, img_width, C, device=dev)
            final_Ts = torch.empty(1, img_height, img_width, device=dev)
            final_idx = torch.empty(1, img_height, img_width, dtype=torch.int32, device=dev)
            with _lib.device_guard(dev):
                _bin_sort(1, N, xys, depths, radii, img_height, img_width, ws, conics, opacity)
                if C == 3:
                    records = _pack_records(1, N, xys, conics, colors, None, opacity)
                    _abi_rasterize_fwd(B=1, N=N, img_h=img_height, img_w=img_width, planar=0, tile_bins=ws.tile_bins,
                                       sorted_ids=ws.sorted_ids, capacity=ws.capacity, records=records, with_extra=0,
                                       background=background, out_img=out_img, final_Ts=final_Ts, final_idx=final_idx)
                else:
                    records = _pack_records(1, N, xys, conics, None, None, opacity)
                    _abi_rasterize_nd_fwd(B=1, N=N, C=C, img_h=img_height, img_w=img_width, tile_bins=ws.tile_bins,
                                          sorted_ids=ws.sorted_ids, capacity=ws.capacity, records=records, colors=colors,
                                          background=background, out_img=out_img, final_Ts=final_Ts, final_idx=final_idx)
            ctx.ws = ws
            ctx.save_for_backward(xys, conics, colors, opacity, background, final_Ts, final_idx, records)
            out_img, final_Ts = out_img[0], final_Ts[0]
        if return_alpha:
            return out_img, 1 - final_Ts
        return out_img

    @staticmethod
    def backward(ctx, v_out_img, v_out_alpha=None):
        saved = ctx.saved_tensors
        xys, conics, colors, opacity, background = saved[:5]
        N = xys.shape[0]
        v_xy = torch.zeros_like(xys)
        v_conic = torch.zeros_like(conics)
        v_colors = torch.zeros_like(colors)
        v_opacity = torch.zeros(N, device=xys.device)
        if ctx.n_isect >= 1 and v_out_img is not None:
            final_Ts, final_idx, records = saved[5], saved[6], saved[7]
            H, W = ctx.dims
            ws = ctx.ws
            va = None if v_out_alpha is None else _f32c(v_out_alpha)
            vo = _f32c(v_out_img)
            with _lib.device_guard(xys.device):
                if colors.shape[-1] == 3:
                    _abi_rasterize_bwd(B=1, N=N, img_h=H, img_w=W, planar=0, tile_bins=ws.tile_bins,
                                       sorted_ids=ws.sorted_ids, capacity=ws.capacity, records=records, with_extra=0,
                                       background=background, final_Ts=final_Ts, final_idx=final_idx, v_out_img=vo,
                                       v_out_alpha=va, v_xy=v_xy, v_conic=v_conic, v_colors=v_colors, v_opacity=v_opacity)
                else:
                    _abi_rasterize_nd_bwd(B=1, N=N, C=colors.shape[-1], img_h=H, img_w=W, tile_bins=ws.tile_bins,
                                          sorted_ids=ws.sorted_ids, capacity=ws.capacity, records=records, colors=colors,
                                          background=background, final_Ts=final_Ts, final_idx=final_idx, v_out_img=vo,
                                          v_out_alpha=va, v_xy=v_xy, v_conic=v_conic, v_colors=v_colors,
                                          v_opacity=v_opacity)
        return (v_xy, None, None, v_conic, None, v_colors, v_opacity[:, None]) + (None,) * 5


def rasterize_gaussians(xys, depths, radii, conics, num_tiles_hit, colors, opacity, img_height, img_width,
                        block_width, background=None, return_alpha=False):
    assert block_width > 1 and block_width <= 16, "block_width must be between 2 and 16"
    if block_width != BLOCK:
        raise NotImplementedError("goliath_amd implements block_width=16 (the reference's value)")
    if colors.dtype == torch.uint8:
        colors = colors.float() / 255
    if xys.ndimension() != 2 or xys.size(1) != 2:
        raise ValueError("xys must have dimensions (N, 2)")
    if colors.ndimension() != 2:
        raise ValueError("colors must have dimensions (N, D)")
    if background is not None:
        assert background.shape[0] == colors.shape[-1], "incorrect shape of background color tensor"
    else:
        background = torch.ones(colors.shape[-1], dtype=torch.float32, device=colors.device)
    if opacity.ndimension() != 2 or opacity.shape[1] != 1:
        opacity = opacity.reshape(-1, 1)
    return _RasterizeGaussians.apply(xys.contiguous(), depths.contiguous(), radii.contiguous(),
                                     conics.contiguous(), num_tiles_hit.contiguous(), colors.contiguous(),
                                     opacity.contiguous(), img_height, img_width, block_width,
                                     background.contiguous(), return_alpha)


class RenderLayout(ctypes.Structure):
    _fields_ = [(n, ctypes.c_int64) for n in (
        "cov3d", "xys", "depths", "radii", "conics", "comp", "nth", "opac_eff", "records", "tile_count", "tile_bins",
        "keys", "sorted_ids", "n_isect", "final_T", "final_idx", "l1_sign", "total")]


_LAYOUTS = {}


def _layout(B, N, img_h, img_w, capacity, with_l1, projected=False):
    key = (B, N, img_h, img_w, capacity, with_l1, projected)
    L = _LAYOUTS.get(key)
    if L is None:
        L = RenderLayout()
        _lib.call("gol_render_layout_projected" if projected else "gol_render_layout", c_int(B), c_int(N), c_int(img_h),
                  c_int(img_w), c_i64(capacity), c_int(with_l1), ctypes.byref(L))
        if len(_LAYOUTS) > 256:
            _LAYOUTS.clear()
        _LAYOUTS[key] = L
    return L


def _ws_view(ws, off, dtype, shape):
    return ws[off:off + math.prod(shape) * dtype.itemsize].view(dtype).view(shape)


def _render_fwd_staged(B, N, src, attrs, background, with_depth, norm_lo, cap, ws, L, out_img, out_depth, alpha, depth_norm,
                       l1_target, l1_mask, l1_mask_c, l1_partial, l1_out, l1_scale):
    a = ws.data_ptr()
    if attrs is not None:
        means, scales, quats, opacity, colors = attrs
        _abi_project_fwd(B=B, N=N, means3d=means, scales=scales, glob_scale=src.glob_scale, quats=quats,
                         viewmats=src.viewmats, intrins=src.intrins, img_h=src.img_h, img_w=src.img_w,
                         clip_thresh=src.clip_thresh, xys=src.xys, depths=src.depths, radii=src.radii, conics=src.conics,
                         compensation=src.comp, opacities=opacity, opac_eff=src.opac_eff, colors=colors,
                         records=src.records)
    _abi_bin_sort(B=B, N=N, xys=src.xys, depths=src.depths, radii=src.radii, conics=src.conics, opacities=src.opac_eff,
                  img_h=src.img_h, img_w=src.img_w, capacity=cap, tile_count=a + L.tile_count, tile_bins=a + L.tile_bins,
                  isect_keys=a + L.keys, sorted_ids=a + L.sorted_ids, n_isect=a + L.n_isect)
    _abi_rasterize_fwd(B=B, N=N, img_h=src.img_h, img_w=src.img_w, planar=1, tile_bins=a + L.tile_bins,
                       sorted_ids=a + L.sorted_ids, capacity=cap, records=src.records, with_extra=int(with_depth),
                       background=background, out_img=out_img, out_extra=out_depth, final_Ts=a + L.final_T,
                       final_idx=a + L.final_idx, out_alpha=alpha, out_extra_norm=depth_norm, norm_lo=norm_lo,
                       l1_target=l1_target, l1_mask=l1_mask, l1_mask_c=l1_mask_c,
                       l1_sign=a + L.l1_sign if l1_target is not None else None, l1_partial=l1_partial, l1_out=l1_out,
                       l1_scale=l1_scale)


def _render_bwd_staged(B, N, src, attrs, grads, background, cap, ws, L, v_img, v_depth, v_alpha, use_l1, l1_mask, v_scale,
                       v_scale_mul, rec):
    a = ws.data_ptr()
    field = lambda k: rec.data_ptr() + 4 * k
    use_depth = v_depth is not None
    rec.zero_()
    _abi_rasterize_bwd(B=B, N=N, img_h=src.img_h, img_w=src.img_w, planar=1, tile_bins=a + L.tile_bins,
                       sorted_ids=a + L.sorted_ids, capacity=cap, records=src.records, with_extra=int(use_depth),
                       background=background, final_Ts=a + L.final_T, final_idx=a + L.final_idx, v_out_img=v_img,
                       v_out_extra=v_depth, v_out_alpha=v_alpha, v_xy=field(4), v_conic=field(6), v_colors=field(0),
                       v_extra=field(9) if use_depth else None, v_opacity=field(3), grad_stride=GRAD_RECORD,
                       v_sign=a + L.l1_sign if use_l1 else None, v_sign_mask=l1_mask,
                       v_sign_mask_c=0 if l1_mask is None else l1_mask.shape[1], v_img_scale=v_scale,
                       v_img_scale_mul=v_scale_mul)
    if attrs is not None:
        means, scales, quats, opacity = attrs
        v_mean, v_scale_g, v_quat, v_opacity = grads
        _abi_project_bwd(B=B, N=N, means3d=means, scales=scales, glob_scale=src.glob_scale, quats=quats,
                         viewmats=src.viewmats, intrins=src.intrins, radii=src.radii, conics=src.conics,
                         compensation=src.comp, v_xy=field(4), v_depth=field(9) if use_depth else None, v_conic=field(6),
                         opacities=opacity, v_opac_eff=field(3), grad_stride=GRAD_RECORD, v_mean3d=v_mean,
                         v_scale=v_scale_g, v_quat=v_quat, v_opacity=v_opacity)


class _RenderViews(torch.autograd.Function):

    @staticmethod
    def forward(ctx, means, scales, quats, opacity, colors, viewmats, intrins, background, img_h, img_w,
                glob_scale, clip_thresh, with_depth, capacity, depth_norm_lo, plan_key, l1_target, l1_mask,
                raw_depth, records, pack, view_set, res):
        projected = records is not None
        B, N = (records if projected else means).shape[:2]
        dev = (records if projected else means).device
        pj = _views.proj_struct(view_set, records, pack) if projected else None
        attrs = None if projected else (means, scales, quats, opacity, colors)
        T = _tiles(img_h, img_w)
        with_l1 = 1 if l1_target is not None else 0
        f = dict(dtype=torch.float32, device=dev)
        out_img = torch.empty(B, 3, img_h, img_w, **f)
        out_depth = torch.empty(B, img_h, img_w, **f) if with_depth and raw_depth else None
        alpha = torch.empty(B, img_h, img_w, **f)
        depth_norm = torch.empty(B, img_h, img_w, **f) if with_depth else None
        l1_partial = torch.empty(B, T, **f) if with_l1 else None
        l1_out = torch.empty(1, **f) if with_l1 else None
        l1_inv_n = 1.0 / max(B * 3 * img_h * img_w, 1)
        l1_mask_c = 0 if l1_mask is None else l1_mask.shape[1]

        def run(cap):
            L = _layout(B, N, img_h, img_w, cap, with_l1, projected)
            ws = torch.empty(max(L.total, 1), dtype=torch.uint8, device=dev)
            a = ws.data_ptr()
            src = pj if projected else _views.ShadeProj(
                fptr(viewmats).value, fptr(intrins).value, img_h, img_w, glob_scale, clip_thresh, a + L.xys, a + L.depths,
                a + L.radii, a + L.conics, a + L.comp, a + L.opac_eff, a + L.records)
            if _lib.TIMING is not None:
                _render_fwd_staged(B, N, src, attrs, background, with_depth, depth_norm_lo, cap, ws, L, out_img, out_depth,
                                   alpha, depth_norm, l1_target, l1_mask, l1_mask_c, l1_partial, l1_out, l1_inv_n)
            else:
                entry = (("gol_render_fwd_projected", c_int(B), c_int(N), ctypes.byref(pj)) if projected else
                         ("gol_render_fwd", c_int(B), c_int(N), c_int(img_h), c_int(img_w), c_float(glob_scale),
                          c_float(clip_thresh), fptr(means), fptr(scales), fptr(quats), fptr(opacity), fptr(colors),
                          fptr(viewmats), fptr(intrins)))
                _lib.call(*entry, fptr(background), c_int(1 if with_depth else 0), c_float(depth_norm_lo), c_i64(cap),
                          ctypes.c_void_p(ws.data_ptr()), ctypes.byref(L), fptr(out_img), fptr(out_depth), fptr(alpha),
                          fptr(depth_norm), fptr(l1_target), fptr(l1_mask), c_int(l1_mask_c), fptr(l1_partial),
                          fptr(l1_out), c_float(l1_inv_n), stream_ptr())
            n_isect = _ws_view(ws, L.n_isect, torch.int32, (B,))
            pending = PLANNER.fetch(n_isect) if plan_key is not None and B > 0 else None
            return ws, L, src, n_isect, pending

        with _lib.device_guard(dev):
            ws, L, src, n_isect, pending = run(capacity)
            if pending is not None:
                worst = PLANNER.finish(*pending)
                if worst > capacity:
                    capacity = PLANNER.set(plan_key, worst)
                    PLANNER.last_worst[plan_key] = worst
                    PLANNER.reruns += 1
                    ws, L, src, n_isect, pending = run(capacity)
                    PLANNER.finish(*pending)
                else:
                    PLANNER.observe(plan_key, worst, capacity)
                PLANNER.passed(plan_key)
        res.bind((B, N, img_h, img_w, T), ws, L, capacity, src, pack if projected else ws, records if projected else ws)
        ctx.L, ctx.capacity, ctx.src = L, capacity, src
        ctx.cfg = (img_h, img_w, glob_scale, with_depth, depth_norm_lo, with_l1)
        ctx.l1_inv_n = l1_inv_n
        l1 = l1_out.reshape(()) if with_l1 else None
        ctx.view_set = view_set
        ctx.save_for_backward(means, scales, quats, opacity, viewmats, intrins, background, ws, l1_mask, records, pack)
        ctx.mark_non_differentiable(ws, n_isect)
        ctx.set_materialize_grads(False)
        return out_img, alpha, out_depth, depth_norm, l1, ws, n_isect

    @staticmethod
    def backward(ctx, v_img, v_alpha, v_depth, v_depth_norm, v_l1, *_non_differentiable):
        means, scales, quats, opacity, viewmats, intrins, background, ws, l1_mask, records, pack = ctx.saved_tensors
        img_h, img_w, glob_scale, with_depth, depth_norm_lo, with_l1 = ctx.cfg
        projected = records is not None
        B, N = (records if projected else means).shape[:2]
        dev = ws.device
        L = ctx.L
        if v_depth_norm is not None:
            final_Ts = _ws_view(ws, L.final_T, torch.float32, (B, img_h, img_w))
            g = v_depth_norm / (1.0 - final_Ts).clamp(depth_norm_lo, 1.0)
            v_depth = g if v_depth is None else v_depth + g
        if not with_l1:
            v_l1 = None
        if v_img is None and v_alpha is None and v_depth is None and v_l1 is None:
            return (None,) * 23
        v_scale = None
        if v_l1 is not None:
            v_scale = v_l1.to(torch.float32).reshape(1).contiguous()
        if v_img is None and v_l1 is None:
            v_img = torch.zeros(B, 3, img_h, img_w, device=dev)
        use_depth = with_depth and v_depth is not None
        v_img_c = None if v_img is None else _f32c(v_img)
        v_depth_c = _f32c(v_depth) if use_depth else None
        v_alpha_c = None if v_alpha is None else _f32c(v_alpha)
        rec = torch.empty(B, N, GRAD_RECORD, device=dev)
        use_mask = l1_mask if v_l1 is not None else None
        attrs = None if projected else (means, scales, quats, opacity)
        grads = None if projected else tuple(torch.empty_like(t) for t in attrs)
        with _lib.device_guard(dev):
            if _lib.TIMING is not None:
                _render_bwd_staged(B, N, ctx.src, attrs, grads, background, ctx.capacity, ws, L, v_img_c, v_depth_c,
                                   v_alpha_c, v_l1 is not None, use_mask, v_scale, ctx.l1_inv_n, rec)
                v_color = None if projected else rec[..., :3]
            else:
                shared = (fptr(background), c_i64(ctx.capacity), ctypes.c_void_p(ws.data_ptr()), ctypes.byref(L),
                          fptr(v_img_c), fptr(v_depth_c), fptr(v_alpha_c), c_int(1 if v_l1 is not None else 0),
                          fptr(use_mask), c_int(0 if use_mask is None else use_mask.shape[1]), fptr(v_scale),
                          c_float(ctx.l1_inv_n), fptr(rec))
                if projected:
                    _lib.call("gol_render_bwd_projected", c_int(B), c_int(N), ctypes.byref(ctx.src), *shared, stream_ptr())
                else:
                    v_color = torch.empty(B, N, 3, device=dev)
                    _lib.call("gol_render_bwd", c_int(B), c_int(N), c_int(img_h), c_int(img_w), c_float(glob_scale),
                              fptr(means), fptr(scales), fptr(quats), fptr(opacity), fptr(viewmats), fptr(intrins), *shared,
                              *(fptr(g) for g in grads), fptr(v_color), stream_ptr())
        if projected:
            return (None,) * 19 + (rec, None, None, None)
        return grads + (v_color,) + (None,) * 18


_BLACK = {}


class _LazyRender(dict):

    def bind(self, dims, ws, L, cap, src, arrays, records):
        self._dims, self._ws, self._L, self._cap, self._src, self._arrays, self._records = dims, ws, L, cap, src, arrays, records

    def __missing__(self, key):
        B, N, H, W, T = self._dims
        ws, L = self._ws, self._L
        if key == "radii":
            buf = self._arrays.view(-1).view(torch.uint8)
            v = _ws_view(buf, (self._src.radii or 0) - buf.data_ptr(), torch.int32, (B, N))
        elif key == "final_T":
            v = _ws_view(ws, L.final_T, torch.float32, (B, 1, H, W))
        elif key == "final_idx":
            v = _ws_view(ws, L.final_idx, torch.int32, (B, H, W))
        elif key == "sorted_ids":
            v = _ws_view(ws, L.sorted_ids, torch.int32, (B, max(self._cap, 1)))
        elif key == "tile_bins":
            v = _ws_view(ws, L.tile_bins, torch.int32, (B, T, 2))
        else:
            raise KeyError(key)
        self[key] = v
        return v


def raster_pair_counts(res):
    B, N, H, W, T = res._dims
    ws, L = res._ws, res._L
    a = ws.data_ptr()
    counts = torch.empty(B, 2, dtype=torch.int64, device=ws.device)
    with _lib.device_guard(ws.device):
        _lib.call("gol_raster_count_pairs", c_int(B), c_int(N), c_int(H), c_int(W), _p(a + L.tile_bins),
                  _p(a + L.sorted_ids), c_i64(res._cap), _p(res._src.records), _p(a + L.final_idx), _p(counts, _I64),
                  stream_ptr())
    return counts


def render_views(means, scales, quats, opacity, colors, viewmats, intrins, img_h, img_w,
                 background=None, glob_scale=1.0, clip_thresh=0.1, with_depth=True, capacity=None, depth_norm_lo=0.05,
                 l1_target=None, l1_mask=None, raw_depth=True, projected=None):
    if projected is not None:
        B, N = projected.records.shape[:2]
        dev = projected.records.device
        if (projected.views.height, projected.views.width) != (img_h, img_w):
            raise ValueError("projected for another image size")
        means = scales = quats = opacity = colors = viewmats = intrins = None
        glob_scale, clip_thresh = projected.views.glob_scale, projected.views.clip_thresh
    else:
        B, N = means.shape[:2]
        dev = means.device
        if not means.is_cuda:
            raise _lib.GoliathHipError("render_views needs CUDA(HIP) tensors; there is no CPU path")
        means, scales, quats, colors = _f32c(means), _f32c(scales), _f32c(quats), _f32c(colors)
        opacity = _f32c(opacity).reshape(B, N)
        viewmats = _f32c(viewmats).reshape(B, viewmats[0].numel() if B else 12)[:, :12].contiguous()
        intrins = _f32c(intrins).reshape(B, 4)
    if background is None:
        background = _BLACK.get(dev)
        if background is None:
            background = _BLACK[dev] = torch.zeros(3, device=dev)
    background = _f32c(background)
    T = _tiles(img_h, img_w)
    key = (B, N, img_h, img_w, dev.index)
    plan_key, deferred = None, False
    if capacity is None:
        planned = PLANNER.get(key)
        if PLANNER.frozen:
            if planned is None:
                raise _lib.GoliathHipError("render_views inside a graph capture needs a calibrated capacity: run the "
                                           "same shapes once eagerly first")
        else:
            if PLANNER.pending:
                PLANNER.poll()
                planned = PLANNER.get(key)
            if planned is None or PLANNER.must_block(key):
                plan_key = key
            else:
                deferred = True
        capacity = planned if planned is not None else PLANNER.initial(N, T)
    if l1_target is not None:
        l1_target = _f32c(l1_target.detach())
        if tuple(l1_target.shape) != (B, 3, img_h, img_w):
            raise ValueError("l1_target must be [B,3,H,W]")
        if l1_mask is not None:
            l1_mask = _f32c(l1_mask.detach())
            if l1_mask.dim() != 4 or l1_mask.shape[0] != B or l1_mask.shape[1] not in (1, 3):
                raise ValueError("l1_mask must be [B,1,H,W] or [B,3,H,W]")
    else:
        l1_mask = None
    res = _LazyRender()
    img, alpha, depth, depth_norm, l1, _, n_isect = _RenderViews.apply(
        means, scales, quats, opacity, colors, viewmats, intrins, background, img_h, img_w, float(glob_scale),
        float(clip_thresh), bool(with_depth), int(capacity), float(depth_norm_lo), plan_key, l1_target, l1_mask,
        bool(raw_depth), None if projected is None else projected.records, None if projected is None else projected.pack,
        None if projected is None else projected.views, res)
    if PLANNER.frozen:
        PLANNER.frozen_log.append((n_isect, res._cap))
    elif deferred and B > 0:
        PLANNER.note(key, n_isect, res._cap)
    res["render"], res["alpha"], res["n_isect"] = img, alpha[:, None], n_isect
    if with_depth:
        if depth is not None:
            res["depth"] = depth[:, None]
        res["depth_norm"] = depth_norm[:, None]
    if l1 is not None:
        res["l1_loss"] = l1
    return res
```

include/goliath_hip.h:

```cpp
#ifndef GOLIATH_HIP_H
#define GOLIATH_HIP_H

#include <stddef.h>
#include <stdint.h>

#ifdef __cplusplus
extern "C" {
#endif

typedef enum {
  GOL_OK = 0,
  GOL_ERR_INVALID_ARG = -1,
  GOL_ERR_LAUNCH = -2,
  GOL_ERR_UNSUPPORTED = -3
} gol_status;

const char* gol_version(void);
const char* gol_last_error(void);
int gol_selftest_wave_sum4(const float* in256, float* out128, void* stream);

int gol_sg_eval_fwd(int N, int D, int L, const float* lobe_dirs, const float* lobe_sigmas,
                    const float* light_values, const float* light_pts, const float* prim_pts,
                    const int32_t* n_lights, float* integral, int w_type, void* stream);
int gol_sg_eval_bwd(int N, int D, int L, const float* lobe_dirs, const float* lobe_sigmas,
                    const float* light_values, const float* light_pts, const float* prim_pts,
                    const int32_t* n_lights, const float* grad_integral, float* grad_dirs,
                    float* grad_sigmas, float* grad_light_values, int w_type, void* stream);

int gol_project_fwd(int B, int N, const float* means3d, const float* scales, float glob_scale,
                    const float* quats, const float* viewmats, const float* intrins, int img_h,
                    int img_w, int block, float clip_thresh, float* cov3d, float* xys,
                    float* depths, int32_t* radii, float* conics, float* compensation,
                    int32_t* num_tiles_hit, const float* opacities, float* opac_eff, const float* colors,
                    float* records, void* stream);
int gol_project_bwd(int B, int N, const float* means3d, const float* scales, float glob_scale,
                    const float* quats, const float* viewmats, const float* intrins,
                    const float* cov3d, const int32_t* radii, const float* conics,
                    const float* compensation, const float* v_xy, const float* v_depth,
                    const float* v_conic, const float* v_compensation, const float* opacities,
                    const float* v_opac_eff, int grad_stride, float* v_mean3d, float* v_scale, float* v_quat,
                    float* v_opacity, void* stream);
int gol_project_bwd_records(int B, int N, const float* means3d, const float* scales, float glob_scale,
                            const float* quats, const float* viewmats, const float* intrins, const int32_t* radii,
                            const float* conics, const float* compensation, const float* opacities,
                            const float* grad_records, int with_depth, float* v_mean3d, float* v_scale, float* v_quat,
                            float* v_opacity, float* v_colors, void* stream);

int gol_bin_sort(int B, int N, const float* xys, const float* depths, const int32_t* radii,
                 const float* conics, const float* opacities, int img_h, int img_w, int block,
                 int64_t capacity, int32_t* tile_count, int32_t* tile_bins, uint64_t* isect_keys,
                 int32_t* sorted_ids, int32_t* n_isect, uint64_t* reach_scratch, void* stream);

#define GOL_GRAD_RECORD 16
#define GOL_SPLAT_RECORD 16
int gol_splat_pack(int B, int N, const float* xys, const float* conics, const float* colors, const float* extra,
                   const float* opacities, float* records, void* stream);
int gol_rasterize_fwd(int B, int N, int img_h, int img_w, int block, int planar, const int32_t* tile_bins,
                      const int32_t* sorted_ids, int64_t capacity, const float* records, int with_extra,
                      const float* background, float* out_img,
                      float* out_extra, float* final_Ts, int32_t* final_idx, float* out_alpha,
                      float* out_extra_norm, float norm_lo, const float* l1_target, const float* l1_mask, int l1_mask_c,
                      uint8_t* l1_sign, float* l1_partial, float* l1_out, float l1_scale, int pixels_per_lane,
                      void* stream);
int gol_rasterize_bwd(int B, int N, int img_h, int img_w, int block, int planar, const int32_t* tile_bins,
                      const int32_t* sorted_ids, int64_t capacity, const float* records, int with_extra,
                      const float* background, const float* final_Ts,
                      const int32_t* final_idx, const float* v_out_img, const float* v_out_extra,
                      const float* v_out_alpha, float* v_xy, float* v_conic, float* v_colors,
                      float* v_extra, float* v_opacity, int grad_stride, const uint8_t* v_sign, const float* v_sign_mask,
                      int v_sign_mask_c, const float* v_img_scale, float v_img_scale_mul, int pixels_per_lane,
                      void* stream);
int gol_raster_count_pairs(int B, int N, int img_h, int img_w, const int32_t* tile_bins, const int32_t* sorted_ids,
                           int64_t capacity, const float* records, const int32_t* final_idx, uint64_t* counts, void* stream);
int gol_raster_plan(int B, int* fwd_pixels_per_lane);

int gol_rasterize_nd_fwd(int B, int N, int C, int img_h, int img_w, int block, const int32_t* tile_bins,
                         const int32_t* sorted_ids, int64_t capacity, const float* records, const float* colors,
                         const float* background, float* out_img, float* final_Ts, int32_t* final_idx,
                         int pixels_per_lane, void* stream);
int gol_rasterize_nd_bwd(int B, int N, int C, int img_h, int img_w, int block, const int32_t* tile_bins,
                         const int32_t* sorted_ids, int64_t capacity, const float* records, const float* colors,
                         const float* background, const float* final_Ts, const int32_t* final_idx,
                         const float* v_out_img, const float* v_out_alpha, float* v_xy, float* v_conic,
                         float* v_colors, float* v_opacity, void* stream);

typedef struct gol_render_ws {
  int64_t cov3d, xys, depths, radii, conics, comp, nth, opac_eff, records, tile_count, tile_bins, keys, sorted_ids,
      n_isect, final_T, final_idx, l1_sign, total;
} gol_render_ws;
int gol_render_layout(int B, int N, int img_h, int img_w, int64_t capacity, int with_l1, gol_render_ws* layout);
int gol_render_fwd(int B, int N, int img_h, int img_w, float glob_scale, float clip_thresh, const float* means,
                   const float* scales, const float* quats, const float* opacity, const float* colors,
                   const float* viewmats, const float* intrins, const float* background, int with_depth, float norm_lo,
                   int64_t capacity, void* workspace, const gol_render_ws* layout, float* out_img, float* out_depth,
                   float* out_alpha, float* out_depth_norm, const float* l1_target, const float* l1_mask, int l1_mask_c,
                   float* l1_partial, float* l1_out, float l1_scale, void* stream);
int gol_render_bwd(int B, int N, int img_h, int img_w, float glob_scale, const float* means, const float* scales,
                   const float* quats, const float* opacity, const float* viewmats, const float* intrins,
                   const float* background, int64_t capacity, void* workspace, const gol_render_ws* layout,
                   const float* v_img, const float* v_depth, const float* v_alpha, int use_l1_sign, const float* l1_mask,
                   int l1_mask_c, const float* v_img_scale, float v_img_scale_mul, float* grad_records, float* v_mean,
                   float* v_scale, float* v_quat, float* v_opacity, float* v_colors, void* stream);

#define GOL_MAX_MIPS 8
typedef struct {
  int32_t B, N;
  int32_t n_color_coef;
  int32_t n_mono_coef;
  const float* f_vnocond;
  const float* f_vcond;
  const float* postex;
  const float* tn;
  const float* albedo;
  const float* light_sh;
  const float* light_sh_rand;
  const float* campos;
  int32_t L;
  const float* light_intensity;
  const float* light_pos;
  const int32_t* n_lights;
  int32_t n_mips;
  const float* mips[GOL_MAX_MIPS];
  int32_t mip_h[GOL_MAX_MIPS], mip_w[GOL_MAX_MIPS];
  const float* lightrot;
  const float* mips_packed[GOL_MAX_MIPS];
  float primscale_min, primscale_max;
  int32_t mips_shared;
  float mips_scale;
} gol_shade_in;

typedef struct {
  float* color;
  float* opacity;
  float* primpos;
  float* primqvec;
  float* primscale;
  float* primscale_preclip;
  float* sigma;
  float* spec_vis;
  float* spec_nml;
  float* spec_dnml;
  float* diff_color;
  float* spec_color;
  float* primnmlbase;
  float* color_rand;
  float* diff_sum;
  float* env_saved;
} gol_shade_out;

typedef struct {
  const float *color, *opacity, *primpos, *primqvec, *primscale, *primscale_preclip, *sigma, *spec_vis,
      *spec_nml, *spec_dnml, *diff_color, *spec_color, *primnmlbase, *color_rand;
} gol_shade_out_grad;

typedef struct {
  float* f_vnocond;
  float* f_vcond;
  float* postex;
  float* tn;
  float* albedo_per_view;
  float* albedo;
} gol_shade_in_grad;

int gol_envmap_pack(int B, int h, int w, const float* src, float* dst, void* stream);
int gol_shade_fwd(const gol_shade_in* in, const gol_shade_out* out, void* stream);
int gol_shade_bwd(const gol_shade_in* in, const gol_shade_out* saved, const gol_shade_out_grad* g,
                  const gol_shade_in_grad* gin, void* stream);

typedef struct {
  const float* viewmats;
  const float* intrins;
  int32_t img_h, img_w;
  float glob_scale, clip_thresh;
  float* xys;
  float* depths;
  int32_t* radii;
  float* conics;
  float* comp;
  float* opac_eff;
  float* records;
} gol_shade_proj;
int gol_shade_project_fwd(const gol_shade_in* in, const gol_shade_out* out, const gol_shade_proj* proj, void* stream);
int gol_render_layout_projected(int B, int N, int img_h, int img_w, int64_t capacity, int with_l1, gol_render_ws* layout);
int gol_render_fwd_projected(int B, int N, const gol_shade_proj* proj, const float* background, int with_depth,
                             float norm_lo, int64_t capacity, void* workspace, const gol_render_ws* layout,
                             float* out_img, float* out_depth, float* out_alpha, float* out_depth_norm,
                             const float* l1_target, const float* l1_mask, int l1_mask_c, float* l1_partial, float* l1_out,
                             float l1_scale, void* stream);
int gol_render_bwd_projected(int B, int N, const gol_shade_proj* proj, const float* background, int64_t capacity,
                             void* workspace, const gol_render_ws* layout, const float* v_img, const float* v_depth,
                             const float* v_alpha, int use_l1_sign, const float* l1_mask, int l1_mask_c,
                             const float* v_img_scale, float v_img_scale_mul, float* grad_records, void* stream);
int gol_shade_project_bwd(const gol_shade_in* in, const gol_shade_out* saved, const gol_shade_out_grad* g,
                          const gol_shade_proj* proj, const float* grad_records, int with_depth,
                          const gol_shade_in_grad* gin, void* stream);

int gol_raydirs_fwd(int N, int H, int W, const float* viewpos, const float* viewrot, const float* focal,
                    const float* princpt, const float* pixelcoords , float volradius,
                    float* raypos, float* raydir, float* tminmax, void* stream);
int gol_mvp_aabb(int N, int K, const float* primpos, const float* primrot, const float* primscale,
                 float* nodeaabb, void* stream);
int gol_mvp_march_fwd(int N, int H, int W, int K, const float* raypos, const float* raydir, float stepsize,
                      const float* tminmax, const float* nodeaabb, const float* primpos,
                      const float* primrot, const float* primscale, const float* tplate, int TD, int TH,
                      int TW, float fadescale, float fadeexp, float* rayrgba, float* raysat, float* shadow,
                      void* stream);
int gol_mvp_march_bwd(int N, int H, int W, int K, const float* raypos, const float* raydir, float stepsize,
                      const float* tminmax, const float* nodeaabb, const float* primpos,
                      const float* primrot, const float* primscale, const float* tplate, int TD, int TH,
                      int TW, float fadescale, float fadeexp, const float* raysat, const float* grad_rayrgba,
                      float* grad_primpos, float* grad_primrot, float* grad_primscale, float* grad_tplate,
                      void* stream);

int gol_mvp_march_warp_fwd(int N, int H, int W, int K, const float* raypos, const float* raydir, float stepsize,
                           const float* tminmax, const float* nodeaabb, const float* primpos,
                           const float* primrot, const float* primscale, const float* tplate, int TD, int TH,
                           int TW, const float* warp, int WD, int WH, int WW, float fadescale, float fadeexp,
                           float* rayrgba, float* raysat, float* shadow, void* stream);
int gol_mvp_march_warp_bwd(int N, int H, int W, int K, const float* raypos, const float* raydir, float stepsize,
                           const float* tminmax, const float* nodeaabb, const float* primpos,
                           const float* primrot, const float* primscale, const float* tplate, int TD, int TH,
                           int TW, const float* warp, int WD, int WH, int WW, float fadescale, float fadeexp,
                           const float* raysat, const float* grad_rayrgba, float* grad_primpos, float* grad_primrot,
                           float* grad_primscale, float* grad_tplate, float* grad_warp, void* stream);

int gol_mvp_shadow_march(int N, int group, int H, int W, int K, const float* raypos, const float* raydir,
                         float stepsize, const float* tminmax, const float* nodeaabb, const float* primpos,
                         const float* primrot, const float* primscale, const float* tplate, int alpha_only,
                         int TD, int TH, int TW, float fadescale, float fadeexp, float* rayrgba, float* shadow,
                         void* stream);

#define GOL_UV_MAX_POW 4
typedef struct {
  int32_t B, L, HW, n_pow;
  float pow[GOL_UV_MAX_POW];
  float fresnel;
  const float *p_uv, *nml, *cam_pos, *light_pos, *light_intensity, *shadow_map, *roughness, *tex_mean;
} gol_uvlight_in;
int gol_uvlight_phong_fwd(const gol_uvlight_in* in, float* diff, float* spec, void* stream);
int gol_uvlight_phong_bwd(const gol_uvlight_in* in, const float* u_diff, const float* u_spec, float* g_p_uv,
                          float* g_nml, void* stream);
int gol_uvlight_ggx_fwd(const gol_uvlight_in* in, float* feat, float* rgb, void* stream);
int gol_uvlight_ggx_bwd(const gol_uvlight_in* in, const float* u_feat, const float* u_rgb, float* g_p_uv,
                        float* g_nml, float* g_roughness, float* g_tex, void* stream);

int gol_l1_blocks(int HW);
int gol_l1_fwd(int B, int C, int HW, int mask_c, const float* pred, const float* target, const float* mask,
               float* partial, void* stream);
int gol_l1_bwd(int B, int C, int HW, int mask_c, const float* pred, const float* target, const float* mask,
               const float* g_loss, float* g_pred, void* stream);

int gol_tail_conv_fwd(int B, int Ci, int h, int w, int CH, int E, int nd, int wB, const float* x, const float* weff,
                      const float* lc, const float* bias, float* out, void* stream);
int gol_tail_conv_bwd(int B, int Ci, int h, int w, int CH, int E, int nd, int wB, const float* x, const float* weff_t,
                      const float* lc, const float* g_out, float* g_x, float* g_weff, float* g_bias, float* w_scratch,
                      void* stream);
long long gol_tail_conv_bwd_scratch_floats(int B, int h, int w, int CH);

int gol_ssim_blocks(int H, int W);
int gol_ssim_fwd(int B, int C, int H, int W, int mask_c, const float* img1, const float* img2, const float* mask,
                 float* partial, float* dmap, void* stream);
int gol_ssim_bwd(int B, int C, int H, int W, const float* img1, const float* img2, const float* dmap,
                 const float* g_scale, float* g_img2, void* stream);

int gol_shadow_pcf(int B, int L, int H, int W, int dh, int dw, const float* depth, const float* Rt, float fx, float fy,
                   float cx, float cy, const float* postex, const float* nml, float exp_scale, float* out,
                   void* stream);

int64_t gol_imgtail_partial_floats(int B, int H, int W);
int gol_imgtail_fwd(int B, int H, int W, const float* rgb, const float* alpha, const float* bg,
                    const float* bg_scale, const float* cal_M, const float* cal_b, const float* blur_w,
                    float* out, void* stream);
int gol_imgtail_bwd(int B, int H, int W, const float* rgb, const float* alpha, const float* bg,
                    const float* bg_scale, const float* cal_M, const float* cal_b, const float* blur_w,
                    const float* g_out, float* g_rgb, float* partials, void* stream);

int64_t gol_mesh_raster_workspace_bytes(int B, int F);
int gol_mesh_raster(int B, int V, int F, int H, int W, const float* v_pix, const int32_t* vi, int32_t* index_img,
                    float* depth_img, float* bary_img, void* workspace, void* stream);

int gol_mesh_render_fwd(int B, int F, int Vt, int C, int H, int W, int Ht, int Wt, const float* vt, const int32_t* vti,
                        const float* tex, const int32_t* index_img, const float* bary_img, float* vt_img, float* render,
                        float* mask, void* stream);
int gol_mesh_render_bwd(int B, int V, int F, int Vt, int C, int H, int W, int Ht, int Wt, const float* v_pix,
                        const int32_t* vi, const float* vt, const int32_t* vti, const float* tex, const int32_t* index_img,
                        const float* bary_img, const float* g_render, const float* g_vt_img, const float* g_bary_img,
                        const float* g_depth_img, float* g_tex, float* g_v_pix, void* stream);
int gol_mesh_render_edge_bwd(int B, int V, int F, int C, int H, int W, const float* v_pix, const int32_t* vi,
                             const int32_t* index_img, const float* depth_img, const float* render,
                             const float* g_render, float* g_v_pix, int32_t* edge_stats, void* stream);

int gol_vert_normals_fwd(int B, int V, int F, const float* verts, const int32_t* vi, const int32_t* vf_start,
                         const int32_t* vf_slot, float eps, float* vn, void* stream);
int gol_vert_normals_bwd(int B, int V, int F, const float* verts, const int32_t* vi, const int32_t* vf_start,
                         const int32_t* vf_slot, float eps, const float* g_vn, float* g_s, float* g_verts, void* stream);
int gol_values_to_uv_fwd(int B, int V, int C, int S, int T, const float* values, const int32_t* texel_rec,
                         const int32_t* triples, float* out, void* stream);
int gol_values_to_uv_bwd(int B, int V, int C, int S, int T, int I, const int32_t* texel_rec, const int32_t* item_start,
                         const int32_t* texel_of, const int32_t* vt_start, const int32_t* vt_slot, const float* g_out,
                         float* item_sums, float* g_values, void* stream);
int gol_uvgeom_fwd(int B, int V, int F, int S, int T, const float* verts, const int32_t* vi, const int32_t* vf_start,
                   const int32_t* vf_slot, const int32_t* texel_rec, const int32_t* triples, float vn_eps, float norm_eps,
                   float* vn, float* postex, float* tn, void* stream);
int gol_uvgeom_bwd(int B, int V, int F, int S, int T, int I, const float* verts, const int32_t* vi,
                   const int32_t* vf_start, const int32_t* vf_slot, const int32_t* texel_rec, const int32_t* triples,
                   const int32_t* item_start, const int32_t* item_tid, const int32_t* texel_of, const int32_t* vt_start,
                   const int32_t* vt_slot, float vn_eps, float norm_eps, const float* vn, const float* g_postex,
                   const float* g_tn, float* item_sums, float* g_s, float* g_verts, void* stream);

int gol_lbs_skeleton_fwd(int B, int J, int NP, int NS, int L, const float* poses, const float* scales, int scales_stride,
                         const float* transform_t, const float* transform_offsets, const float* joint_offset,
                         const float* joint_rotation, const double* bind_inv, const int32_t* parents,
                         const int32_t* level_start, const int32_t* level_joints, float* states, float* mats,
                         void* stream);
int gol_lbs_skeleton_bwd(int B, int J, int NP, int NS, int L, const float* poses, const float* scales, int scales_stride,
                         const float* transform, const float* transform_t, const float* transform_offsets,
                         const float* joint_offset, const float* joint_rotation, const double* bind_inv,
                         const int32_t* parents, const int32_t* level_start, const int32_t* level_joints,
                         const int32_t* child_start, const int32_t* child_slot, const float* g_states,
                         const float* g_mats, float* g_poses, float* g_scales, void* stream);
int gol_lbs_skin_fwd(int B, int V, int J, int K, const float* mats, const float* verts, int verts_batched,
                     const float* template_verts, const float* global_scaling, const int32_t* skin_indices,
                     const float* skin_weights, float* out, void* stream);
int gol_lbs_skin_bwd(int B, int V, int J, int K, int E, int I, const float* mats, const float* verts, int verts_batched,
                     const float* template_verts, const float* global_scaling, const int32_t* skin_indices,
                     const float* skin_weights, const int32_t* item_start, const int32_t* jv_slot,
                     const int32_t* ji_start, const float* g_out, double* item_sums, float* g_verts, float* g_mats,
                     void* stream);

#define GOL_OPTIM_GROUP_DOUBLES 8
#define GOL_OPTIM_SCRUB 1
#define GOL_OPTIM_CLIP 2
#define GOL_OPTIM_WRITE_BACK 4
int gol_optim_chunk_elems(void);
int gol_optim_grad_stats(int n_chunks, int n_seg, const int32_t* chunk_seg, const int64_t* chunk_off, const int64_t* seg_g,
                         const int64_t* seg_numel, double* partial, void* stream);
int gol_optim_finalize(int n_chunks, const double* partial, double max_norm, double* stats, int64_t* nonfinite,
                       void* stream);
int gol_optim_adam_step(int n_chunks, int n_seg, int n_groups, const int32_t* chunk_seg, const int64_t* chunk_off,
                        const int64_t* seg_p, const int64_t* seg_g, const int64_t* seg_m, const int64_t* seg_v,
                        const int64_t* seg_step, const int64_t* seg_numel, const int32_t* seg_group, const double* groups,
                        const double* stats, float* seg_coef, int flags, void* stream);

typedef enum {
  GOL_REGLOSS_BOUND = 0,
  GOL_REGLOSS_NEG_SQ = 1,
  GOL_REGLOSS_SQ = 2,
  GOL_REGLOSS_ABS = 3,
  GOL_REGLOSS_ALPHAPRIOR = 4
} gol_regloss_kind;
int gol_regloss_chunk_elems(void);
int gol_regloss_fwd(int kind, int64_t n, float p0, float p1, const float* x, double* partial, void* stream);
int gol_regloss_bwd(int kind, int64_t n, float p0, float p1, const float* x, const float* g_scale, float* g_x,
                    void* stream);
int gol_backlit_fwd(int64_t m, int c, const float* color, const float* cosw, double* partial, void* stream);
int gol_backlit_bwd(int64_t m, int c, const float* color, const float* cosw, const float* g_scale, float* g_color,
                    void* stream);

#ifdef __cplusplus
}
#endif
#endif
```

Baseline: 2955 views/s.

## Record per-wave taker masks in forward and reuse them to prune backward visits

The forward raster kernel now records, for each tile entry, which half-tiles (wave groups) actually composited that Gaussian, and writes one byte per entry into a new workspace buffer. The backward kernel reads these bytes instead of recomputing the geometric wave mask, so it skips Gaussians that were culled by alpha or transmittance as well as those outside the region. It also specializes the backward visit on whether opacity caps alpha and whether the start-index check is needed, and folds the uncapped opacity scaling into the merge weights. Adding waves_per_eu hints to the forward kernel is a separate occupancy change. In exchange the forward pass does extra ballots, shared-memory and global byte writes, and needs a capacity-sized buffer per view.

```diff
diff --git a/goliath_amd/csrc/gol_raster.h b/goliath_amd/csrc/gol_raster.h
--- a/goliath_amd/csrc/gol_raster.h
+++ b/goliath_amd/csrc/gol_raster.h
@@ -81,7 +81,7 @@
 struct __attribute__((aligned(16))) StagedRow { float4 a, b; float2 c; float2 pad; };
 
 struct Staged { float4 a, b; float2 c; int mask; };
-template <int PPL>
+template <int PPL, bool MASK = true>
 __device__ __forceinline__ Staged stage_entry(const float* __restrict__ records, size_t g, float tile_x0, float tile_y0) {
   const float4* R = reinterpret_cast<const float4*>(records + g * GOL_SPLAT_RECORD);
   const float4 q0 = R[0], q1 = R[1], q2 = R[2], q3 = R[3];
@@ -90,8 +90,13 @@
   s.b = q1;
   s.c = make_float2(q2.x, q2.y);
   const float3 cn = true_conic(q0.z, q0.w, q1.x);
-  s.mask = wave_mask<PPL>(q0.x, q0.y, cn.x, cn.y, cn.z, q2.z, q2.w, q3.x, q3.y, tile_x0, tile_y0);
+  s.mask = MASK ? wave_mask<PPL>(q0.x, q0.y, cn.x, cn.y, cn.z, q2.z, q2.w, q3.x, q3.y, tile_x0, tile_y0) : 0;
   return s;
+}
+
+template <int PPL> __device__ __forceinline__ int taker_half(int wave) { return PPL == 2 ? wave : wave >> 1; }
+template <int PPL> __device__ __forceinline__ int taker_wave_mask(int rec) {
+  return PPL == 2 ? (rec & 3) : ((rec & 1) ? 3 : 0) | ((rec & 2) ? 12 : 0);
 }
 
 template <typename V, int P>
@@ -121,7 +126,8 @@
 template <int PPL>
 __device__ __forceinline__ unsigned long long fwd_step(const fvec<PPL>& sigma, fvec<PPL> alpha, const fvec<PPL>& live,
                                                        const fvec<PPL>& T_cur, fvec<PPL>& vis, fvec<PPL>& next_T,
-                                                       bool (&take)[PPL], unsigned long long (&stop)[PPL]) {
+                                                       bool (&take)[PPL], unsigned long long (&stop)[PPL],
+                                                       unsigned long long& any_take) {
   alpha *= live;
   vis = alpha * T_cur;
 #ifndef GOL_EXACT_MATH
@@ -131,11 +137,13 @@
   for (int q = 0; q < PPL; ++q) next_T[q] = exact_next_T(T_cur[q], alpha[q]);
 #endif
   unsigned long long any_stop = 0ull;
+  any_take = 0ull;
 #pragma unroll
   for (int q = 0; q < PPL; ++q) {
     const unsigned long long mc = gol_ballot(!(sigma[q] < 0.f)) & gol_ballot(!(alpha[q] < GOL_ALPHA_FLOOR));
     const unsigned long long ms = gol_ballot(next_T[q] <= GOL_T_STOP);
     take[q] = __builtin_amdgcn_inverse_ballot_w64(mc & ~ms);
+    any_take |= mc & ~ms;
     stop[q] = mc & ms;
     any_stop |= stop[q];
   }
@@ -154,7 +162,7 @@
 #endif
 }
 
-template <int PPL>
+template <int PPL, bool CAP = true, bool START = true>
 __device__ __forceinline__ unsigned long long bwd_taken(float opacity, const fvec<PPL>& e, const fvec<PPL>& sigma, int li,
                                                         const ivec<PPL>& bin_final, fvec<PPL>& alpha,
                                                         unsigned long long (&mv)[PPL]) {
@@ -162,8 +170,9 @@
   unsigned long long many = 0ull;
 #pragma unroll
   for (int q = 0; q < PPL; ++q) {
-    alpha[q] = fminf(GOL_ALPHA_CAP_BWD, alpha[q]);
-    mv[q] = gol_ballot(li <= bin_final[q]) & gol_ballot(!(sigma[q] < 0.f)) & gol_ballot(!(alpha[q] < GOL_ALPHA_FLOOR));
+    if (CAP) alpha[q] = fminf(GOL_ALPHA_CAP_BWD, alpha[q]);
+    mv[q] = gol_ballot(!(sigma[q] < 0.f)) & gol_ballot(!(alpha[q] < GOL_ALPHA_FLOOR));
+    if (START) mv[q] &= gol_ballot(li <= bin_final[q]);
     many |= mv[q];
   }
   return many;
@@ -185,19 +194,29 @@
   T_cur = T_new;
 }
 
-template <int PPL>
-__device__ __forceinline__ void bwd_moments(const fvec<PPL>& e, const fvec<PPL>& w, const fvec<PPL>& T_cur,
-                                            const fvec<PPL>& ra, const fvec<PPL>& fac, const fvec<PPL>& tail,
-                                            const bool (&v)[PPL], const fvec<PPL>& dy, fvec<PPL>& qsum, fvec<PPL>& gop,
-                                            fvec<PPL>& gy, fvec<PPL>& gyy) {
+template <int PPL, bool CAP = true>
+__device__ __forceinline__ void bwd_moments(const fvec<PPL>& e, const fvec<PPL>& alpha, const fvec<PPL>& w,
+                                            const fvec<PPL>& T_cur, const fvec<PPL>& ra, const fvec<PPL>& fac,
+                                            const fvec<PPL>& tail, const bool (&v)[PPL], const fvec<PPL>& dy, fvec<PPL>& qsum,
+                                            fvec<PPL>& gop, fvec<PPL>& gy, fvec<PPL>& gyy, float gop_scale = 1.f) {
   const fvec<PPL> v_alpha = T_cur * w + ra * (tail - qsum);
   qsum += fac * w;
-  gop = e * v_alpha;
-#pragma unroll
-  for (int q = 0; q < PPL; ++q) gop[q] = v[q] ? gop[q] : 0.f;
+  if (CAP) {
+    gop = (e * gop_scale) * v_alpha;
+#pragma unroll
+    for (int q = 0; q < PPL; ++q) gop[q] = v[q] ? gop[q] : 0.f;
+  } else {
+    gop = alpha * v_alpha;
+  }
   gy = gop * dy;
   gyy = gy * dy;
 }
+__device__ __forceinline__ bool bwd_capped(float opacity) { return !(opacity <= GOL_ALPHA_CAP_BWD); }
+__device__ __forceinline__ void bwd_merge_weights(float opacity, float& wop, float& wsig) {
+  const bool capped = bwd_capped(opacity);
+  wop = capped ? 1.f : 1.f / opacity;
+  wsig = capped ? -opacity : -1.f;
+}
 template <int PPL>
 __device__ __forceinline__ float lane_sum(const fvec<PPL>& x) {
   float s = x[0];
@@ -214,6 +233,16 @@
 #pragma unroll
   for (int off = 32; off > 0; off >>= 1) wmax = max(wmax, __shfl_xor(wmax, off, 64));
   return __builtin_amdgcn_readfirstlane(wmax);
+}
+
+template <int PPL>
+__device__ __forceinline__ int wave_first_final(const ivec<PPL>& bin_final) {
+  int wmin = bin_final[0];
+#pragma unroll
+  for (int q = 1; q < PPL; ++q) wmin = min(wmin, bin_final[q]);
+#pragma unroll
+  for (int off = 32; off > 0; off >>= 1) wmin = min(wmin, __shfl_xor(wmin, off, 64));
+  return __builtin_amdgcn_readfirstlane(wmin);
 }
 
 inline int64_t raster_grid(int B, int img_h, int img_w) {
diff --git a/goliath_amd/csrc/raster.hip b/goliath_amd/csrc/raster.hip
--- a/goliath_amd/csrc/raster.hip
+++ b/goliath_amd/csrc/raster.hip
@@ -2,21 +2,23 @@
 
 #include "gol_raster.h"
 
+
 namespace {
 
 template <bool EXTRA, bool LAZY, int PPL>
-__global__ __launch_bounds__(64 * Pix<PPL>::kWaves) void raster_fwd_kernel(
+__global__ __launch_bounds__(64 * Pix<PPL>::kWaves) __attribute__((amdgpu_waves_per_eu(PPL == 2 ? 6 : 7))) void raster_fwd_kernel(
     int N, int img_h, int img_w, int planar, int tiles_x, int tiles_y, const int2* __restrict__ tile_bins,
     const int32_t* __restrict__ sorted_ids, int64_t capacity, const float* __restrict__ records,
     const float* __restrict__ background, float* __restrict__ out_img,
     float* __restrict__ out_extra, float* __restrict__ final_Ts, int32_t* __restrict__ final_idx,
     float* __restrict__ out_alpha, float* __restrict__ out_extra_norm, float norm_lo,
     const float* __restrict__ l1_target, const float* __restrict__ l1_mask, int l1_mask_c,
-    uint8_t* __restrict__ l1_sign, float* __restrict__ l1_partial, int n_views) {
+    uint8_t* __restrict__ l1_sign, float* __restrict__ l1_partial, uint8_t* __restrict__ takers, int n_views) {
   typedef typename Pix<PPL>::fv fv;
   typedef typename Pix<PPL>::iv iv;
   constexpr int NW = Pix<PPL>::kWaves, NT = 64 * NW;
   __shared__ float s_l1[NW];
+  __shared__ unsigned long long s_take[2][NW][kBatch / 64];
   __shared__ float4 s_a[kBatch];
   __shared__ float4 s_b[kBatch];
   __shared__ float2 s_c[kBatch];
@@ -47,9 +49,24 @@
   fv acc0 = 0.f, acc1 = 0.f, acc2 = 0.f, acc3 = 0.f;
 
   const int n_batches = (range.y - range.x + kBatch - 1) / kBatch;
-  for (int bb = 0; bb < n_batches; ++bb) {
-    if (__syncthreads_and(!any_live<fv, PPL>(live))) break;
+  uint8_t* __restrict__ o_take = takers ? takers + (size_t)view * capacity : nullptr;
+  auto store_takers = [&](int b) {
+    for (int k = tid; k < kBatch; k += NT) {
+      const int idx = range.x + b * kBatch + k;
+      if (idx >= range.y) break;
+      unsigned rec = 0u;
+#pragma unroll
+      for (int w = 0; w < NW; ++w) rec |= (unsigned)((s_take[b & 1][w][k >> 6] >> (k & 63)) & 1ull) << taker_half<PPL>(w);
+      o_take[idx] = (uint8_t)rec;
+    }
+  };
+  int bb = 0;
+  for (; bb < n_batches; ++bb) {
+    const bool finished = __syncthreads_and(!any_live<fv, PPL>(live));
+    if (o_take && bb > 0) store_takers(bb - 1);
+    if (finished) break;
     const int batch_start = range.x + bb * kBatch;
+    if (tid < NW * (kBatch / 64)) (&s_take[bb & 1][0][0])[tid] = 0ull;
     for (int k = tid; k < kBatch; k += NT) {
       const int idx = batch_start + k;
       if (idx < range.y) {
@@ -64,9 +81,12 @@
     for (int chunk = 0; chunk < batch_size; chunk += 64) {
       unsigned long long bits = gol_ballot((s_mask[chunk + lane] >> wave) & 1);
       if (LAZY && gol_ballot(any_live<fv, PPL>(live)) == 0ull) break;
+      const int chunk_id = chunk >> 6;
+      unsigned long long taken_bits = 0ull;
       while (bits) {
         if (!LAZY && gol_ballot(any_live<fv, PPL>(live)) == 0ull) { chunk = batch_size; break; }
-        const int t = chunk + __builtin_ctzll(bits);
+        const int tb = __builtin_ctzll(bits);
+        const int t = chunk + tb;
         bits &= bits - 1;
         const float4 a4 = s_a[t];
         const float4 b4 = s_b[t];
@@ -78,8 +98,9 @@
 #pragma unroll
         for (int q = 0; q < PPL; ++q) alpha[q] = fminf(GOL_ALPHA_CAP_FWD, b4.y * e[q]);
         bool take[PPL];
-        unsigned long long stop_m[PPL];
-        const unsigned long long any_stop = fwd_step<PPL>(sigma, alpha, live, T_cur, vis, next_T, take, stop_m);
+        unsigned long long stop_m[PPL], any_take;
+        const unsigned long long any_stop = fwd_step<PPL>(sigma, alpha, live, T_cur, vis, next_T, take, stop_m, any_take);
+        taken_bits |= any_take != 0ull ? 1ull << tb : 0ull;
         bool half_done = false;
         if (!LAZY || any_stop != 0ull) {
 #pragma unroll
@@ -99,7 +120,11 @@
         }
         if (LAZY && half_done) { chunk = batch_size; break; }
       }
-    }
+      if (o_take && taken_bits != 0ull && lane == 0) s_take[bb & 1][wave][chunk_id] = taken_bits;
+    }
+  }
+  if (o_take && n_batches > 0) {
+    if (bb == n_batches) { __syncthreads(); store_takers(n_batches - 1); }
   }
   if (LAZY) {
 #pragma unroll
@@ -203,7 +228,7 @@
     const float* __restrict__ v_out_alpha, float* __restrict__ v_xy, float* __restrict__ v_conic,
     float* __restrict__ v_colors, float* __restrict__ v_extra, float* __restrict__ v_opacity,
     const uint8_t* __restrict__ v_sign, const float* __restrict__ v_sign_mask, int v_sign_mask_c,
-    const float* __restrict__ v_img_scale, float v_img_scale_mul, int n_views) {
+    const float* __restrict__ v_img_scale, float v_img_scale_mul, const uint8_t* __restrict__ takers, int n_views) {
   typedef typename Pix<PPL>::fv fv;
   typedef typename Pix<PPL>::iv iv;
   constexpr int NW = Pix<PPL>::kWaves, NT = 64 * NW;
@@ -270,7 +295,7 @@
   const fv tail = T_final * (voa - (background[0] * vo0 + background[1] * vo1 + background[2] * vo2));
   fv qsum = 0.f;
 
-  const int wmax = wave_last_entry<PPL>(bin_final);
+  const int wmax = wave_last_entry<PPL>(bin_final), wmin = wave_first_final<PPL>(bin_final);
   if (lane == 0) s_wmax[wave] = wmax;
   __syncthreads();
   int bmax = s_wmax[0];
@@ -285,31 +310,41 @@
     const int e = bmax - bb2 * kBatchB - tid;
     return (tid < kBatchB && e >= range.x) ? ids[e] : 0;
   };
-  int gid_next = entry_id(0);
+  const uint8_t* __restrict__ i_take = takers ? takers + (size_t)view * capacity : nullptr;
+  auto entry_takers = [&](int bb2) {
+    const int e = bmax - bb2 * kBatchB - tid;
+    return (i_take && tid < kBatchB && e >= range.x) ? (int)i_take[e] : 0;
+  };
+  int gid_next = entry_id(0), rec_next = entry_takers(0);
   for (int bb = 0; bb < n_batches; ++bb) {
     __syncthreads();
     const int batch_end = bmax - bb * kBatchB;
     const int batch_size = min(kBatchB, batch_end + 1 - range.x);
-    const int gid = gid_next;
+    const int gid = gid_next, rec = rec_next;
     if (tid < kBatchB) {
       if (tid < batch_size) {
-        const Staged st = stage_entry<PPL>(records, goff + (size_t)gid, (float)(tc.tx * 16), (float)(tc.ty * 16));
-        s_e[tid].a = st.a; s_e[tid].b = st.b; s_e[tid].c = st.c; s_mask[tid] = st.mask;
+        if (i_take) {
+          const Staged st = stage_entry<PPL, false>(records, goff + (size_t)gid, 0.f, 0.f);
+          s_e[tid].a = st.a; s_e[tid].b = st.b; s_e[tid].c = st.c; s_mask[tid] = taker_wave_mask<PPL>(rec);
+        } else {
+          const Staged st = stage_entry<PPL>(records, goff + (size_t)gid, (float)(tc.tx * 16), (float)(tc.ty * 16));
+          s_e[tid].a = st.a; s_e[tid].b = st.b; s_e[tid].c = st.c; s_mask[tid] = st.mask;
+        }
         s_id[tid] = gid;
       } else {
         s_mask[tid] = 0;
       }
     }
-    if (bb + 1 < n_batches) gid_next = entry_id(bb + 1);
+    if (bb + 1 < n_batches) { gid_next = entry_id(bb + 1); rec_next = entry_takers(bb + 1); }
     (&s_touched[0][0])[tid] = 0;
     __syncthreads();
 
     const int t0 = max(0, batch_end - wmax);
     unsigned long long bits = gol_ballot((s_mask[lane] >> wave) & 1);
     if (t0 > 0) bits &= ~0ull << t0;
-    while (bits) {
-      const int t = __builtin_ctzll(bits);
-      bits &= bits - 1;
+    const unsigned long long cap_bits = gol_ballot(bwd_capped(s_e[lane].b.y));
+    auto visit = [&](int t, auto cap_c, auto start_c) {
+      constexpr bool CAP = decltype(cap_c)::value, START = decltype(start_c)::value;
       const float4 a4 = s_e[t].a;
       const float4 b4 = s_e[t].b;
       const float2 c2 = s_e[t].c;
@@ -319,13 +354,13 @@
       fv sigma, vis, alpha, ra, fac;
       visit_falloff<PPL>(a4.z, a4.w, b4.x, dx, dy, sigma, vis);
       unsigned long long mv[PPL];
-      if (bwd_taken<PPL>(b4.y, vis, sigma, li, bin_final, alpha, mv) == 0ull) continue;
+      if (bwd_taken<PPL, CAP, START>(b4.y, vis, sigma, li, bin_final, alpha, mv) == 0ull) return;
       bool v[PPL];
       bwd_recur<PPL>(mv, alpha, T_cur, v, ra, fac);
       fv w = b4.z * vo0 + b4.w * vo1 + c2.x * vo2;
       if (EXTRA) w += c2.y * vo3;
       fv gop, gy, gyy;
-      bwd_moments<PPL>(vis, w, T_cur, ra, fac, tail, v, dy, qsum, gop, gy, gyy);
+      bwd_moments<PPL, CAP>(vis, alpha, w, T_cur, ra, fac, tail, v, dy, qsum, gop, gy, gyy, bwd_capped(b4.y) ? 1.f : b4.y);
       float g0s, g1s, g2s, g3 = 0.f;
       if (PPL == 2) {
         g0s = __builtin_fmaf(fac[0], vo0[0], fac[PPL - 1] * vo0[PPL - 1]);
@@ -348,7 +383,13 @@
         if (lane == 63) { a[8 - 3] = r2; a[9 - 3] = r3; }
         s_touched[wave][t] = 1;
       }
-    }
+    };
+    auto walk = [&](auto cap_c, auto start_c) {
+      for (unsigned long long b = bits; b; b &= b - 1) visit(__builtin_ctzll(b), cap_c, start_c);
+    };
+    if (bits & cap_bits) walk(kYes, kYes);
+    else if (batch_end - t0 > wmin) walk(kNo, kYes);
+    else walk(kNo, kNo);
     __syncthreads();
     if (PACKED) {
       float* rec = v_colors;
@@ -360,10 +401,12 @@
         if (!any || c > (EXTRA ? 9 : 8)) continue;
         const float4 a4 = s_e[t].a;
         const float4 b4 = s_e[t].b;
-        const float nop = -b4.y, cc = b4.x;
+        const float cc = b4.x;
+        float wop = 1.f, nop = -b4.y;
+        bwd_merge_weights(b4.y, wop, nop);
         const int k1 = (c == 5) ? 4 : c, k2 = 5;
         const float w1 = (c == 4) ? nop * a4.z * kUnA : (c == 5) ? nop * a4.w * kUnB : (c == 6 || c == 8) ? 0.5f * nop
-                       : (c == 7) ? nop : 1.f;
+                       : (c == 7) ? nop : (c == 3) ? wop : 1.f;
         const float w2 = (c == 4) ? nop * a4.w * kUnB : (c == 5) ? nop * cc * kUnA : 0.f;
         float s1 = 0.f, s2 = 0.f;
 #pragma unroll
@@ -394,10 +437,11 @@
         const size_t g = goff + (size_t)s_id[tid];
         const float4 a4 = s_e[tid].a;
         const float4 b4 = s_e[tid].b;
-        const float nop = -b4.y;
+        float wop = 1.f, nop = -b4.y;
+        bwd_merge_weights(b4.y, wop, nop);
         const float3 cn = true_conic(a4.z, a4.w, b4.x);
         atomicAdd(v_colors + 3 * g, a[0]); atomicAdd(v_colors + 3 * g + 1, a[1]); atomicAdd(v_colors + 3 * g + 2, a[2]);
-        atomicAdd(v_opacity + g, a[3]);
+        atomicAdd(v_opacity + g, wop * a[3]);
         atomicAdd(v_xy + 2 * g, nop * (cn.x * a[4] + cn.y * a[5]));
         atomicAdd(v_xy + 2 * g + 1, nop * (cn.y * a[4] + cn.z * a[5]));
         atomicAdd(v_conic + 3 * g, 0.5f * nop * a[6]); atomicAdd(v_conic + 3 * g + 1, nop * a[7]);
@@ -500,7 +544,7 @@
                                  float* out_extra, float* final_Ts, int32_t* final_idx, float* out_alpha,
                                  float* out_extra_norm, float norm_lo, const float* l1_target, const float* l1_mask,
                                  int l1_mask_c, uint8_t* l1_sign, float* l1_partial, float* l1_out, float l1_scale,
-                                 int pixels_per_lane, void* stream) {
+                                 uint8_t* takers, int pixels_per_lane, void* stream) {
   GOL_RASTER_CHECK_DIMS(12, "image too large (32-bit byte offsets inside a view)");
   if (B == 0) return GOL_OK;
   GOL_REQUIRE(tile_bins && background && out_img && final_Ts && final_idx, "null pointer");
@@ -525,7 +569,7 @@
       raster_fwd_kernel<EX, LZ, PPL><<<grid, 64 * Pix<PPL>::kWaves, 0, s>>>(
           N, img_h, img_w, planar, tiles_x, tiles_y, bins, sorted_ids, capacity, records, background, out_img, out_extra,
           final_Ts, final_idx, out_alpha, EX ? out_extra_norm : nullptr, norm_lo, l1_target, l1_mask, l1_mask_c, l1_sign,
-          l1_partial, B);
+          l1_partial, takers, B);
     });
   };
   const bool ex = out_extra || out_extra_norm;
@@ -545,7 +589,7 @@
                                  const float* v_out_alpha, float* v_xy, float* v_conic, float* v_colors,
                                  float* v_extra, float* v_opacity, int grad_stride, const uint8_t* v_sign,
                                  const float* v_sign_mask, int v_sign_mask_c, const float* v_img_scale,
-                                 float v_img_scale_mul, int pixels_per_lane, void* stream) {
+                                 float v_img_scale_mul, const uint8_t* takers, int pixels_per_lane, void* stream) {
   GOL_RASTER_CHECK_DIMS(0, "");
   if (B == 0 || N == 0 || capacity == 0) return GOL_OK;
   GOL_REQUIRE(tile_bins && sorted_ids && background && final_Ts && final_idx, "null pointer");
@@ -575,7 +619,7 @@
       raster_bwd_kernel<EX, PK, PPL><<<grid, 64 * Pix<PPL>::kWaves, 0, s>>>(
           N, img_h, img_w, planar, tiles_x, tiles_y, bins, sorted_ids, capacity, records, background, final_Ts, final_idx,
           v_out_img, EX ? v_out_extra : nullptr, v_out_alpha, v_xy, v_conic, v_colors, EX ? v_extra : nullptr, v_opacity,
-          v_sign, v_sign_mask, v_sign_mask_c, v_img_scale, v_img_scale_mul, B);
+          v_sign, v_sign_mask, v_sign_mask_c, v_img_scale, v_img_scale_mul, takers, B);
     });
   };
   if (ex && packed) launch(kYes, kYes);
diff --git a/goliath_amd/csrc/raster_nd.hip b/goliath_amd/csrc/raster_nd.hip
--- a/goliath_amd/csrc/raster_nd.hip
+++ b/goliath_amd/csrc/raster_nd.hip
@@ -88,7 +88,8 @@
         for (int q = 0; q < PPL; ++q) alpha[q] = fminf(GOL_ALPHA_CAP_FWD, b2.y * e[q]);
         bool take[PPL];
         unsigned long long stop_m[PPL];
-        fwd_step<PPL>(sigma, alpha, live, T_cur, vis, next_T, take, stop_m);
+        unsigned long long any_take;
+        fwd_step<PPL>(sigma, alpha, live, T_cur, vis, next_T, take, stop_m, any_take);
 #pragma unroll
         for (int q = 0; q < PPL; ++q) live[q] = __builtin_amdgcn_inverse_ballot_w64(stop_m[q]) ? 0.f : live[q];
         fwd_take<PPL>(take, next_T, vis, T_cur);
@@ -237,7 +238,7 @@
 #pragma unroll
       for (int c = 0; c < CK; ++c) w += col[c] * vo[c];
       fv gop, gy, gyy;
-      bwd_moments<PPL>(vis, w, T_cur, ra, fac, tail, v, dy, qsum, gop, gy, gyy);
+      bwd_moments<PPL>(vis, alpha, w, T_cur, ra, fac, tail, v, dy, qsum, gop, gy, gyy);
       float s[kRow];
 #pragma unroll
       for (int c = 0; c < CK; ++c) {
diff --git a/goliath_amd/csrc/render.hip b/goliath_amd/csrc/render.hip
--- a/goliath_amd/csrc/render.hip
+++ b/goliath_amd/csrc/render.hip
@@ -31,6 +31,7 @@
   L->final_T = take((int64_t)B * P * 4);
   L->final_idx = take((int64_t)B * P * 4);
   L->l1_sign = with_l1 ? take((int64_t)B * P) : -1;
+  L->takers = take((int64_t)B * cap);
   L->total = o;
   return GOL_OK;
 }
@@ -58,8 +59,8 @@
                            capacity, records, with_depth ? 1 : 0, background, out_img,
                            with_depth ? out_depth : nullptr, at<float>(ws, L->final_T), at<int32_t>(ws, L->final_idx),
                            out_alpha, with_depth ? out_depth_norm : nullptr, norm_lo, l1_target, l1_mask, l1_mask_c,
-                           l1_target ? at<uint8_t>(ws, L->l1_sign) : nullptr, l1_partial, l1_out, l1_scale, 0,
-                           stream);
+                           l1_target ? at<uint8_t>(ws, L->l1_sign) : nullptr, l1_partial, l1_out, l1_scale,
+                           at<uint8_t>(ws, L->takers), 0, stream);
 }
 
 static int render_bwd_to_records(int B, int N, int img_h, int img_w, const float* records, const float* background,
@@ -79,7 +80,7 @@
                            at<float>(ws, L->final_T), at<int32_t>(ws, L->final_idx), v_img, v_depth, v_alpha, g + 4, g + 6,
                            g, use_depth ? g + 9 : nullptr, g + 3, GOL_GRAD_RECORD,
                            use_l1_sign ? at<uint8_t>(ws, L->l1_sign) : nullptr, use_l1_sign ? l1_mask : nullptr,
-                           use_l1_sign ? l1_mask_c : 0, v_img_scale, v_img_scale_mul, 0, stream);
+                           use_l1_sign ? l1_mask_c : 0, v_img_scale, v_img_scale_mul, at<uint8_t>(ws, L->takers), 0, stream);
 }
 
 extern "C" int gol_render_fwd(int B, int N, int img_h, int img_w, float glob_scale, float clip_thresh, const float* means,
diff --git a/goliath_amd/splat.py b/goliath_amd/splat.py
--- a/goliath_amd/splat.py
+++ b/goliath_amd/splat.py
@@ -178,23 +178,24 @@
 def _abi_rasterize_fwd(*, B, N, img_h, img_w, planar, tile_bins, sorted_ids, capacity, records, with_extra, background,
                        out_img, out_extra=None, final_Ts, final_idx, out_alpha=None, out_extra_norm=None, norm_lo=0.0,
                        l1_target=None, l1_mask=None, l1_mask_c=0, l1_sign=None, l1_partial=None, l1_out=None,
-                       l1_scale=1.0, pixels_per_lane=0):
+                       l1_scale=1.0, takers=None, pixels_per_lane=0):
     _lib.call("gol_rasterize_fwd", c_int(B), c_int(N), c_int(img_h), c_int(img_w), c_int(BLOCK), c_int(planar),
               _p(tile_bins, _I32), _p(sorted_ids, _I32), c_i64(capacity), _p(records), c_int(with_extra),
               _p(background), _p(out_img), _p(out_extra), _p(final_Ts), _p(final_idx, _I32), _p(out_alpha),
               _p(out_extra_norm), c_float(norm_lo), _p(l1_target), _p(l1_mask), c_int(l1_mask_c), _p(l1_sign, _U8),
-              _p(l1_partial), _p(l1_out), c_float(l1_scale), c_int(pixels_per_lane), stream_ptr())
+              _p(l1_partial), _p(l1_out), c_float(l1_scale), _p(takers, _U8), c_int(pixels_per_lane), stream_ptr())
 
 
 def _abi_rasterize_bwd(*, B, N, img_h, img_w, planar, tile_bins, sorted_ids, capacity, records, with_extra, background,
                        final_Ts, final_idx, v_out_img=None, v_out_extra=None, v_out_alpha=None, v_xy, v_conic, v_colors,
                        v_extra=None, v_opacity, grad_stride=0, v_sign=None, v_sign_mask=None, v_sign_mask_c=0,
-                       v_img_scale=None, v_img_scale_mul=1.0, pixels_per_lane=0):
+                       v_img_scale=None, v_img_scale_mul=1.0, takers=None, pixels_per_lane=0):
     _lib.call("gol_rasterize_bwd", c_int(B), c_int(N), c_int(img_h), c_int(img_w), c_int(BLOCK), c_int(planar),
               _p(tile_bins, _I32), _p(sorted_ids, _I32), c_i64(capacity), _p(records), c_int(with_extra), _p(background),
               _p(final_Ts), _p(final_idx, _I32), _p(v_out_img), _p(v_out_extra), _p(v_out_alpha), _p(v_xy), _p(v_conic),
               _p(v_colors), _p(v_extra), _p(v_opacity), c_int(grad_stride), _p(v_sign, _U8), _p(v_sign_mask),
-              c_int(v_sign_mask_c), _p(v_img_scale), c_float(v_img_scale_mul), c_int(pixels_per_lane), stream_ptr())
+              c_int(v_sign_mask_c), _p(v_img_scale), c_float(v_img_scale_mul), _p(takers, _U8), c_int(pixels_per_lane),
+              stream_ptr())
 
 
 def _abi_rasterize_nd_fwd(*, B, N, C, img_h, img_w, tile_bins, sorted_ids, capacity, records, colors, background, out_img,
@@ -391,7 +392,7 @@
 class RenderLayout(ctypes.Structure):
     _fields_ = [(n, ctypes.c_int64) for n in (
         "cov3d", "xys", "depths", "radii", "conics", "comp", "nth", "opac_eff", "records", "tile_count", "tile_bins",
-        "keys", "sorted_ids", "n_isect", "final_T", "final_idx", "l1_sign", "total")]
+        "keys", "sorted_ids", "n_isect", "final_T", "final_idx", "l1_sign", "takers", "total")]
 
 
 _LAYOUTS = {}
@@ -433,7 +434,7 @@
                        final_idx=a + L.final_idx, out_alpha=alpha, out_extra_norm=depth_norm, norm_lo=norm_lo,
                        l1_target=l1_target, l1_mask=l1_mask, l1_mask_c=l1_mask_c,
                        l1_sign=a + L.l1_sign if l1_target is not None else None, l1_partial=l1_partial, l1_out=l1_out,
-                       l1_scale=l1_scale)
+                       l1_scale=l1_scale, takers=a + L.takers)
 
 
 def _render_bwd_staged(B, N, src, attrs, grads, background, cap, ws, L, v_img, v_depth, v_alpha, use_l1, l1_mask, v_scale,
@@ -449,7 +450,7 @@
                        v_extra=field(9) if use_depth else None, v_opacity=field(3), grad_stride=GRAD_RECORD,
                        v_sign=a + L.l1_sign if use_l1 else None, v_sign_mask=l1_mask,
                        v_sign_mask_c=0 if l1_mask is None else l1_mask.shape[1], v_img_scale=v_scale,
-                       v_img_scale_mul=v_scale_mul)
+                       v_img_scale_mul=v_scale_mul, takers=a + L.takers)
     if attrs is not None:
         means, scales, quats, opacity = attrs
         v_mean, v_scale_g, v_quat, v_opacity = grads
@@ -603,6 +604,8 @@
             v = _ws_view(ws, L.sorted_ids, torch.int32, (B, max(self._cap, 1)))
         elif key == "tile_bins":
             v = _ws_view(ws, L.tile_bins, torch.int32, (B, T, 2))
+        elif key == "takers":
+            v = _ws_view(ws, L.takers, torch.uint8, (B, max(self._cap, 1)))
         else:
             raise KeyError(key)
         self[key] = v
diff --git a/include/goliath_hip.h b/include/goliath_hip.h
--- a/include/goliath_hip.h
+++ b/include/goliath_hip.h
@@ -60,16 +60,16 @@
                       const float* background, float* out_img,
                       float* out_extra, float* final_Ts, int32_t* final_idx, float* out_alpha,
                       float* out_extra_norm, float norm_lo, const float* l1_target, const float* l1_mask, int l1_mask_c,
-                      uint8_t* l1_sign, float* l1_partial, float* l1_out, float l1_scale, int pixels_per_lane,
-                      void* stream);
+                      uint8_t* l1_sign, float* l1_partial, float* l1_out, float l1_scale, uint8_t* takers,
+                      int pixels_per_lane, void* stream);
 int gol_rasterize_bwd(int B, int N, int img_h, int img_w, int block, int planar, const int32_t* tile_bins,
                       const int32_t* sorted_ids, int64_t capacity, const float* records, int with_extra,
                       const float* background, const float* final_Ts,
                       const int32_t* final_idx, const float* v_out_img, const float* v_out_extra,
                       const float* v_out_alpha, float* v_xy, float* v_conic, float* v_colors,
                       float* v_extra, float* v_opacity, int grad_stride, const uint8_t* v_sign, const float* v_sign_mask,
-                      int v_sign_mask_c, const float* v_img_scale, float v_img_scale_mul, int pixels_per_lane,
-                      void* stream);
+                      int v_sign_mask_c, const float* v_img_scale, float v_img_scale_mul, const uint8_t* takers,
+                      int pixels_per_lane, void* stream);
 int gol_raster_count_pairs(int B, int N, int img_h, int img_w, const int32_t* tile_bins, const int32_t* sorted_ids,
                            int64_t capacity, const float* records, const int32_t* final_idx, uint64_t* counts, void* stream);
 int gol_raster_plan(int B, int* fwd_pixels_per_lane);
@@ -86,7 +86,7 @@
 
 typedef struct gol_render_ws {
   int64_t cov3d, xys, depths, radii, conics, comp, nth, opac_eff, records, tile_count, tile_bins, keys, sorted_ids,
-      n_isect, final_T, final_idx, l1_sign, total;
+      n_isect, final_T, final_idx, l1_sign, takers, total;
 } gol_render_ws;
 int gol_render_layout(int B, int N, int img_h, int img_w, int64_t capacity, int with_l1, gol_render_ws* layout);
 int gol_render_fwd(int B, int N, int img_h, int img_w, float glob_scale, float clip_thresh, const float* means,
```

Measured after the change: 2961 views/s, median of 5. No clear change (+0.2%).
